# NAIVEddd/MafrixRaytracing

Hardware: AMD Instinct MI355X
Metric: Mrays/s (primary+secondary) at 1080p/64spp; 1/2/4/8-GPU scaling (higher is better)
Workload: dtype f64; 1 GPU; C2 spot (5856 tris) + floor/light stage, 1920x1080, 64 spp per step over 1 GPU(s); scene=scenes/spot.xml, width=1920, height=1080, max_depth=3, frames_in_flight=1, pipeline=wavefront, api=mfx_trace_accumulate of the step's spp (inputs resident in HBM), parallelism=one GPU

## Files before the change

mafrixraytracing_amd/csrc/cut_check.cpp:

```cpp
#include <algorithm>
#include <cfloat>
#include <cinttypes>
#include <cmath>
#include <cstdio>
#include <cstdlib>
#include <cstring>
#include <string>
#include <vector>

#include "mfx_build.h"
#include "mfx_camera_cuts.h"
#include "mfx_scene.h"

hipError_t mfx_gpu_build_images(const float*, const float*, const int32_t*, int, int, float, const MfxGpuLayoutIn&,
                                MfxGpuImages&) {
    return hipErrorNotSupported;
}

namespace {

struct Rng {
    uint64_t x;
    uint64_t next() {
        uint64_t z = (x += 0x9e3779b97f4a7c15ULL);
        z = (z ^ (z >> 30)) * 0xbf58476d1ce4e5b9ULL;
        z = (z ^ (z >> 27)) * 0x94d049bb133111ebULL;
        return z ^ (z >> 31);
    }
    double unit() { return (double)(next() >> 11) * 0x1p-53; }
    double in(double lo, double hi) { return lo + (hi - lo) * unit(); }
};

const double ALBEDO[9] = {0.75, 0.25, 0.25, 0.25, 0.75, 0.25, 0.5, 0.5, 0.5};

mfx_pinhole pinhole(double px, double py, double pz, double dx, double dy, double dz, double fov) {
    mfx_pinhole c;
    std::memset(&c, 0, sizeof(c));
    c.position[0] = px; c.position[1] = py; c.position[2] = pz;
    c.direction[0] = dx; c.direction[1] = dy; c.direction[2] = dz;
    c.fov = fov;
    c.aspect = 16.0 / 9.0;
    return c;
}

mfx_scene_desc desc_of(const std::vector<mfx_prim>& prims, const mfx_pinhole& cam) {
    mfx_scene_desc d;
    std::memset(&d, 0, sizeof(d));
    d.prims = prims.data();
    d.nprims = (int64_t)prims.size();
    d.albedo = ALBEDO;
    d.nmat = 3;
    d.width = 40;
    d.height = 24;
    d.max_depth = 3;
    const double q[4][3] = {{-0.5, 2.5, -0.5}, {0.5, 2.5, -0.5}, {0.5, 2.5, 0.5}, {-0.5, 2.5, 0.5}};
    std::memcpy(d.light.p, q, sizeof(q));
    d.light.normal[1] = -1.0;
    d.light.intensity[0] = d.light.intensity[1] = d.light.intensity[2] = 3.0;
    d.camera = cam;
    return d;
}

std::vector<mfx_prim> soup(int n, uint64_t seed) {
    Rng r{seed};
    std::vector<mfx_prim> v(n);
    for (int i = 0; i < n; ++i) {
        mfx_prim& p = v[i];
        std::memset(&p, 0, sizeof(p));
        p.material = i % 3;
        const double x = r.in(-1.0, 1.0), y = r.in(-1.0, 1.0), z = r.in(-1.0, 1.0);
        if (i % 3 == 0) {
            p.kind = MFX_PRIM_TRIANGLE;
            const double c[3] = {x, y, z};
            for (int k = 0; k < 3; ++k)
                for (int a = 0; a < 3; ++a) p.p[k][a] = c[a] + (k ? r.in(-0.05, 0.05) : 0.0);
        } else if (i % 3 == 1) {
            p.kind = MFX_PRIM_RECT;
            const double u = r.in(0.02, 0.1), w = r.in(0.02, 0.1), t = r.in(-0.03, 0.03);
            const double q[4][3] = {{x, y, z}, {x + u, y, z + t}, {x + u, y + w, z + t}, {x, y + w, z}};
            std::memcpy(p.p, q, sizeof(q));
        } else {
            p.kind = MFX_PRIM_SPHERE;
            p.p[0][0] = x; p.p[0][1] = y; p.p[0][2] = z;
            p.p[1][0] = r.in(0.01, 0.08);
        }
    }
    return v;
}

bool load_prims(const char* path, std::vector<mfx_prim>& v) {
    FILE* f = std::fopen(path, "rb");
    if (!f) return false;
    std::fseek(f, 0, SEEK_END);
    const long bytes = std::ftell(f);
    std::fseek(f, 0, SEEK_SET);
    if (bytes <= 0 || bytes % (long)sizeof(mfx_prim) != 0) {
        std::fclose(f);
        return false;
    }
    v.resize((size_t)bytes / sizeof(mfx_prim));
    const size_t got = std::fread(v.data(), sizeof(mfx_prim), v.size(), f);
    std::fclose(f);
    return got == v.size();
}

struct RayF {
    float ix, iy, iz, oix, oiy, oiz;
};
RayF make_rayf(const double* o, const double* d) {
    float dx = (float)d[0], dy = (float)d[1], dz = (float)d[2];
    const float tiny = 1e-20f;
    if (std::fabs(dx) < tiny) dx = std::copysign(tiny, dx);
    if (std::fabs(dy) < tiny) dy = std::copysign(tiny, dy);
    if (std::fabs(dz) < tiny) dz = std::copysign(tiny, dz);
    RayF r;
    r.ix = 1.0f / dx; r.iy = 1.0f / dy; r.iz = 1.0f / dz;
    r.oix = (float)o[0] * r.ix; r.oiy = (float)o[1] * r.iy; r.oiz = (float)o[2] * r.iz;
    return r;
}
bool slab(const MfxNode& nd, int k, const RayF& r, float& n) {
    const float a0 = std::fmaf(nd.lox[k], r.ix, -r.oix), a1 = std::fmaf(nd.hix[k], r.ix, -r.oix);
    const float b0 = std::fmaf(nd.loy[k], r.iy, -r.oiy), b1 = std::fmaf(nd.hiy[k], r.iy, -r.oiy);
    const float c0 = std::fmaf(nd.loz[k], r.iz, -r.oiz), c1 = std::fmaf(nd.hiz[k], r.iz, -r.oiz);
    n = std::fmax(std::fmax(std::fmin(a0, a1), std::fmin(b0, b1)), std::fmax(std::fmin(c0, c1), 0.0f));
    const float f = std::fmin(std::fmin(std::fmax(a0, a1), std::fmax(b0, b1)), std::fmin(std::fmax(c0, c1), FLT_MAX));
    return n <= f;
}

struct Totals {
    long long rays = 0, leaves = 0, uncovered = 0, lb_above = 0, tiles = 0, root = 0, empty = 0, multi = 0;
};

int find_entry(const MfxCutEntry* row, int cap, int code) {
    for (int i = 0; i < cap && row[i].code != MFX_CUT_END; ++i)
        if (row[i].code == code) return i;
    return -1;
}

void check_ray(const std::vector<MfxNode>& nodes, const RayF& r, const MfxCutEntry* row, int cap, Totals& t) {
    struct Item {
        int node, cov;
    };
    std::vector<Item> stack{{0, find_entry(row, cap, 0)}};
    while (!stack.empty()) {
        const Item it = stack.back();
        stack.pop_back();
        const MfxNode& nd = nodes[it.node];
        for (int k = 0; k < 4; ++k) {
            if (nd.child[k] == MFX_CHILD_EMPTY) continue;
            float n = 0.f;
            if (!slab(nd, k, r, n)) continue;
            int cov = it.cov;
            if (cov < 0) {
                cov = find_entry(row, cap, nd.child[k]);
                if (cov >= 0 && !(row[cov].lb <= n)) ++t.lb_above;
            }
            if (nd.child[k] >= 0) {
                stack.push_back({nd.child[k], cov});
            } else {
                ++t.leaves;
                if (cov < 0) ++t.uncovered;
            }
        }
    }
}

void check_case(const char* scene, const char* camname, const MfxHostScene& s, const MfxCamera& cam, int W, int H, int cap,
                Totals& all, double* root_share = nullptr) {
    const int tiles_x = (W + 7) / 8, tiles_y = (H + 7) / 8;
    std::vector<MfxCutEntry> table((size_t)tiles_x * tiles_y * cap);
    MfxCutStats st;
    mfx_cut::table_host(s.nodes.data(), cam, W, H, cap, table.data(), st);
    Totals t;
    t.tiles = (long long)tiles_x * tiles_y;
    t.root = (long long)st.root_tiles;
    t.empty = (long long)st.empty_tiles;
    for (int n = 2; n <= MFX_CUT_CAP_MAX; ++n) t.multi += (long long)st.hist[n];
    Rng jr{(uint64_t)(W * 131 + H * 7 + cap)};
    const double one = 1.0 - 0x1p-53;
    for (int y = 0; y < H; ++y)
        for (int x = 0; x < W; ++x) {
            const MfxCutEntry* row = table.data() + (size_t)((y / 8) * tiles_x + x / 8) * cap;
            for (int j = 0; j < 16; ++j) {
                const double ju = j < 4 ? ((j & 1) ? one : 0.0) : jr.unit(), jv = j < 4 ? ((j & 2) ? one : 0.0) : jr.unit();
                const double u = ((double)x + ju) / (double)W, v = ((double)y + jv) / (double)H;
                double o[3], d[3];
                for (int a = 0; a < 3; ++a) {
                    o[a] = cam.position[a];
                    d[a] = ((cam.topleft[a] + cam.right[a] * u) + cam.down[a] * v) - o[a];
                }
                const double l = std::sqrt(d[0] * d[0] + d[1] * d[1] + d[2] * d[2]);
                if (l != 0.0)
                    for (int a = 0; a < 3; ++a) d[a] = d[a] / l;
                ++t.rays;
                check_ray(s.nodes, make_rayf(o, d), row, cap, t);
            }
        }
    std::printf("%s %s %dx%d cap=%d: tiles=%lld root=%lld empty=%lld multi=%lld mean_len=%.3f max_len=%llu rays=%lld leaves=%lld"
                " uncovered=%lld lb_above=%lld\n",
                scene, camname, W, H, cap, t.tiles, t.root, t.empty, t.multi, (double)st.len_sum / (double)t.tiles, st.len_max,
                t.rays, t.leaves, t.uncovered, t.lb_above);
    if (root_share) *root_share = (double)t.root / (double)t.tiles;
    all.rays += t.rays; all.leaves += t.leaves; all.uncovered += t.uncovered; all.lb_above += t.lb_above;
    all.tiles += t.tiles; all.root += t.root; all.empty += t.empty; all.multi += t.multi;
}

bool build(const std::vector<mfx_prim>& prims, const mfx_pinhole& cam, MfxHostScene& s) {
    const mfx_scene_desc d = desc_of(prims, cam);
    std::string err;
    if (!mfx_build_scene(&d, s, err)) {
        std::printf("build FAILED: %s\n", err.c_str());
        return false;
    }
    return true;
}

struct NamedCam {
    const char* name;
    mfx_pinhole cam;
};

std::vector<NamedCam> cameras(const mfx_pinhole& def, const MfxHostScene& s) {
    double c[3], R = 0.0;
    for (int a = 0; a < 3; ++a) {
        c[a] = 0.5 * (s.box_lo[a] + s.box_hi[a]);
        R = std::max(R, 0.5 * (s.box_hi[a] - s.box_lo[a]));
    }
    const double* p = def.position;
    const double* d = def.direction;
    const double dl = std::sqrt(d[0] * d[0] + d[1] * d[1] + d[2] * d[2]);
    return {{"default", def},
            {"inside", pinhole(c[0], c[1], c[2], d[0], d[1], d[2], 90.0)},
            {"away", pinhole(p[0], p[1], p[2], -d[0], -d[1], -d[2], 90.0)},
            {"axis", pinhole(c[0], c[1], c[2] + 3.0 * R, 0.0, 0.0, -1.0, 90.0)},
            {"far_0.6deg", pinhole(c[0] - 200.0 * R * d[0] / dl, c[1] - 200.0 * R * d[1] / dl, c[2] - 200.0 * R * d[2] / dl, d[0],
                                   d[1], d[2], 0.6)},
            {"fov120", pinhole(p[0], p[1], p[2], d[0], d[1], d[2], 120.0)}};
}

int check_scene(const char* name, const std::vector<mfx_prim>& prims, const mfx_pinhole& def, bool cap_root_share, Totals& all) {
    MfxHostScene s;
    if (!build(prims, def, s)) return 1;
    int bad = 0;
    for (const NamedCam& nc : cameras(def, s)) {
        MfxCamera cam;
        mfx_derive_camera(nc.cam, cam);
        const int films[2][2] = {{40, 24}, {17, 9}};
        for (const auto& f : films)
            for (const int cap : {MFX_CUT_CAP_DEFAULT, 1, 2, MFX_CUT_CAP_MAX}) {
                double share = 0.0;
                check_case(name, nc.name, s, cam, f[0], f[1], cap, all, &share);
                if (cap_root_share && cap == MFX_CUT_CAP_DEFAULT && std::strcmp(nc.name, "default") == 0) {
                    std::printf("%s default %dx%d: {root} share %.4f (cap 0.05)\n", name, f[0], f[1], share);
                    if (share > 0.05) {
                        std::printf("FAIL: {root} share above 5 %%\n");
                        ++bad;
                    }
                }
            }
    }
    return bad;
}

int distribution(const std::vector<mfx_prim>& prims, const mfx_pinhole& def, int W, int H) {
    MfxHostScene s;
    if (!build(prims, def, s)) return 1;
    MfxCamera cam;
    mfx_derive_camera(def, cam);
    const int tiles = ((W + 7) / 8) * ((H + 7) / 8);
    for (const int cap : {MFX_CUT_CAP_MAX, MFX_CUT_CAP_DEFAULT}) {
        std::vector<MfxCutEntry> table((size_t)tiles * cap);
        MfxCutStats st;
        mfx_cut::table_host(s.nodes.data(), cam, W, H, cap, table.data(), st);
        long long internal = 0, entries = 0;
        for (const MfxCutEntry& e : table)
            if (e.code != MFX_CUT_END) {
                ++entries;
                internal += e.code >= 0;
            }
        std::printf("%dx%d cap=%d nodes=%zu tiles=%d mean=%.3f max=%llu root=%llu empty=%llu internal_entries=%.4f hist:", W, H, cap,
                    s.nodes.size(), tiles, (double)st.len_sum / tiles, st.len_max, st.root_tiles, st.empty_tiles,
                    entries ? (double)internal / (double)entries : 0.0);
        for (int n = 0; n <= cap; ++n) std::printf(" %d:%llu", n, st.hist[n]);
        std::printf("\n");
    }
    return 0;
}

}

int main(int argc, char** argv) {
    const mfx_pinhole spot_cam = pinhole(2.4, 1.3, -3.4, -2.4, -1.2, 3.4, 90.0);
    const mfx_pinhole soup_cam = pinhole(0.0, 0.0, 4.5, 0.0, 0.0, -1.0, 90.0);
    std::vector<mfx_prim> mesh;
    if (argc > 1 && !load_prims(argv[1], mesh)) {
        std::printf("cannot read %s\n", argv[1]);
        return 2;
    }
    if (argc == 4) return distribution(mesh, spot_cam, std::atoi(argv[2]), std::atoi(argv[3]));
    if (argc == 11) {
        double v[7];
        for (int i = 0; i < 7; ++i) v[i] = std::atof(argv[4 + i]);
        return distribution(mesh, pinhole(v[0], v[1], v[2], v[3], v[4], v[5], v[6]), std::atoi(argv[2]), std::atoi(argv[3]));
    }
    Totals all;
    int bad = check_scene("soup_600", soup(600, 600), soup_cam, false, all);
    if (!mesh.empty()) bad += check_scene("mesh", mesh, spot_cam, true, all);
    std::printf("total: rays=%lld leaves=%lld uncovered=%lld lb_above=%lld tiles=%lld root=%lld empty=%lld multi=%lld\n", all.rays,
                all.leaves, all.uncovered, all.lb_above, all.tiles, all.root, all.empty, all.multi);
    if (all.uncovered || all.lb_above) {
        std::printf("FAIL: a reached leaf is not covered, or an entry's lb is above a ray's entry distance\n");
        ++bad;
    }
    if (all.empty == 0 || all.multi == 0 || all.leaves == 0) {
        std::printf("FAIL: vacuous (no empty cut, no cut of more than one entry, or no leaf reached)\n");
        ++bad;
    }
    return bad ? 1 : 0;
}
```

mafrixraytracing_amd/csrc/mfx_api.cpp:

```cpp
#include <dlfcn.h>

#include <set>
#include <thread>

#include "mfx_ctx.h"
#include "mfx_half.h"

using namespace mfxh;

namespace {
thread_local std::string g_err;

using mfx_half::node_to_half;

template <typename T>
hipError_t upload(DevBuf<T>& d, const std::vector<T>& v) {
    const hipError_t e = d.alloc(std::max<size_t>(1, v.size()));
    if (e != hipSuccess || v.empty()) return e;
    return hipMemcpy(d, v.data(), v.size() * sizeof(T), hipMemcpyHostToDevice);
}
}

int mfxh::fail(int code, const std::string& msg) {
    g_err = msg;
    return code;
}

const Rccl* mfxh::rccl() {
    static Rccl r;
    static bool tried = false, ok = false;
    if (tried) return ok ? &r : nullptr;
    tried = true;
    void* h = dlopen("librccl.so.1", RTLD_NOW | RTLD_GLOBAL);
    if (!h) h = dlopen("/opt/rocm/lib/librccl.so.1", RTLD_NOW | RTLD_GLOBAL);
    if (!h) return nullptr;
    r.commInitAll = (decltype(r.commInitAll))dlsym(h, "ncclCommInitAll");
    r.commDestroy = (decltype(r.commDestroy))dlsym(h, "ncclCommDestroy");
    r.reduce = (decltype(r.reduce))dlsym(h, "ncclReduce");
    r.groupStart = (decltype(r.groupStart))dlsym(h, "ncclGroupStart");
    r.groupEnd = (decltype(r.groupEnd))dlsym(h, "ncclGroupEnd");
    r.errorString = (decltype(r.errorString))dlsym(h, "ncclGetErrorString");
    ok = r.commInitAll && r.commDestroy && r.reduce && r.groupStart && r.groupEnd && r.errorString;
    return ok ? &r : nullptr;
}

int mfxh::whole_film_single_device(const mfx_ctx* c, const char* who) {
    if (c->api_part_count != 1 || (c->flags & MFX_F_ROW_PARTITION) || c->multi.device_list || !c->multi.peers.empty())
        return fail(MFX_E_STATE, std::string(who) + " needs one device and the whole film and sample set "
                                                    "(no device list, part_count == 1, no MFX_F_ROW_PARTITION)");
    return MFX_OK;
}

mfx_ctx::~mfx_ctx() {
    for (ncclComm_t cm : multi.comms)
        if (cm) (void)rccl()->commDestroy(cm);
    multi.comms.clear();
    multi.peers.clear();
    (void)hipSetDevice(device);
}

static CreateEnv read_create_env() {
    const auto set = [](const char* name) { return getenv(name) != nullptr; };
    const auto num = [](const char* name) { return getenv(name) ? CreateEnv::Int(atoi(getenv(name))) : std::nullopt; };
    CreateEnv v;
    v.node_f32 = set("MFX_NODE_F32");
    v.diag_iter = set("MFX_DIAG_ITER");
    v.no_gray_light = set("MFX_NO_GRAY_LIGHT");
    v.no_lit_in_hit = set("MFX_NO_LIT_IN_HIT");
    v.mega_waves = num("MFX_MEGA_WAVES");
    v.shadow_target_blocks = num("MFX_SHADOW_TARGET_BLOCKS");
    v.stack_lds = num("MFX_STACK_LDS");
    v.ntop = num("MFX_NTOP");
    v.slot_lds = num("MFX_SLOT_LDS");
    v.shadow_waves = num("MFX_SHADOW_WAVES");
    v.blocks_per_cu = num("MFX_BLOCKS_PER_CU");
    v.camera_packets = num("MFX_CAMERA_PACKETS");
    v.cam_blocks = num("MFX_CAM_BLOCKS");
    v.camera_cuts = num("MFX_CAMERA_CUTS");
    v.camera_cut_cap = num("MFX_CAMERA_CUT_CAP");
    v.camera_cut_min_samples = num("MFX_CAMERA_CUT_MIN_SAMPLES");
    v.pool_fail_once = num("MFX_POOL_FAIL_ONCE");
    v.adaptive_check = num("MFX_ADAPTIVE_CHECK");
    v.iter_events = num("MFX_ITER_EVENTS");
    v.queue_from = num("MFX_QUEUE_FROM");
    v.qchunk = num("MFX_QCHUNK");
    v.ray_queue = num("MFX_RAY_QUEUE");
    v.mega_chunk = num("MFX_MEGA_CHUNK");
    v.shd_half = num("MFX_SHD_HALF");
    v.chunk = num("MFX_CHUNK");
    if (const char* e = getenv("MFX_POOL")) v.pool = atoll(e);
    return v;
}

template <typename F>
static int largest_keeping(int lo, int hi, F keeps) {
    while (lo < hi) {
        const int mid = (lo + hi + 1) / 2;
        if (keeps(mid)) lo = mid;
        else hi = mid - 1;
    }
    return lo;
}

#define CK(expr) HIP_TRY(expr, _e == hipErrorOutOfMemory ? MFX_E_NOMEM : MFX_E_DEVICE, #expr ": ")

static int scene_upload(mfx_ctx* c) {
    c->image_gen += 1;
    c->stack_size = std::max(1, c->host.stack_entries);
    if (c->stack_size > 96) return fail(MFX_E_INVALID, "mfx_create: BVH too deep for the LDS traversal stack");
    CK(upload(c->d_nodes, c->host.nodes));
    CK(upload(c->d_slots, c->host.slots));
    if (MFX_NODE_F16 && !c->env.node_f32) {
        std::vector<MfxNodeH> nh(c->host.nodes.size());
        for (size_t i = 0; i < nh.size(); ++i) nh[i] = node_to_half(c->host.nodes[i]);
        CK(upload(c->d_nodes_h, nh));
    }
    CK(upload(c->d_slot_ref, c->host.slot_ref));
    CK(upload(c->d_ref_blob, c->host.ref_blob));
    CK(upload(c->d_shade, c->host.shade));
    CK(upload(c->d_albedo, c->host.albedo));
    CK(upload(c->d_light, std::vector<MfxLight>{c->host.light}));
    if (wf_multi_light(c)) CK(upload(c->d_lights, c->host.lights));
    else c->d_lights.reset();
    CK(upload(c->d_cam, std::vector<MfxCamera>{c->host.camera}));
    CK(upload(c->d_refs, std::vector<const void*>{c->d_slot_ref.get(), c->d_ref_blob.get()}));
    if (!c->host.inst.empty()) CK(upload(c->d_inst, c->host.inst));
    else c->d_inst.reset();
    return MFX_OK;
}

static int scene_shapes(mfx_ctx* c) {
    const CreateEnv& env = c->env;
    const bool inst = !c->host.inst.empty();
    hipDeviceProp_t prop;
    CK(hipGetDeviceProperties(&prop, c->device));
    int bpc = 0;
    c->mega_waves = c->stack_size <= 36 ? 4 : 1;
    if (env.mega_waves) c->mega_waves = *env.mega_waves == 4 ? 4 : 1;
    CK(mfx_trace_occupancy(c->stack_size, &bpc, inst, c->mega_waves));
    bpc = std::max(1, std::min(bpc, 8));
    c->grid = prop.multiProcessorCount * bpc;
    WfParams& A = c->pool.params;
    hipError_t qerr = hipSuccess;
    auto blocks = [&](bool shd, int nlds, int ntop = 0, int nslot = 0) {
        const WfLdsShape s{shd, nlds < c->stack_size, c->d_nodes_h != nullptr, nlds, ntop, (int)c->host.inst.size(), nslot,
                           shd && wf_multi_light(c)};
        int b = 0;
        const hipError_t e = mfx_wf_kernel_occupancy(s, &b);
        if (e != hipSuccess && qerr == hipSuccess) qerr = e;
        return e == hipSuccess ? b : 0;
    };
    int ebpc = 0, sbpc = 0;
    for (const bool shd : {false, true}) {
        const int full = blocks(shd, c->stack_size);
        int nlds = c->stack_size;
        if (c->stack_size > WF_STACK_LDS) {
            const int b16 = blocks(shd, WF_STACK_LDS);
            const int target = shd ? std::max(full, std::min(env.shadow_target_blocks.value_or(8), b16)) : b16;
            if (full < target) nlds = largest_keeping(WF_STACK_LDS, c->stack_size - 1, [&](int n) { return blocks(shd, n) >= target; });
            if (c->diag_iter)
                fprintf(stderr, "wavefront: %s blocks/CU: full %d-entry stacks %d, %d in LDS %d; chosen %d in LDS, %d\n",
                        shd ? "k_shadow" : "k_extend", c->stack_size, full, WF_STACK_LDS, b16, nlds, blocks(shd, nlds));
        }
        if (env.stack_lds) nlds = std::max(1, std::min(c->stack_size, *env.stack_lds));
        (shd ? A.stack_lds_shd : A.stack_lds_ext) = nlds;
        (shd ? sbpc : ebpc) = blocks(shd, nlds);
    }
    {
        int cap = std::min((int)c->host.nodes.size(), WF_NTOP_MAX);
        if (env.ntop) cap = std::max(0, std::min(cap, *env.ntop));
        for (const bool shd : {false, true}) {
            const int nlds = shd ? A.stack_lds_shd : A.stack_lds_ext, want = shd ? sbpc : ebpc;
            const int ntop = largest_keeping(0, cap, [&](int n) { return blocks(shd, nlds, n) >= want; });
            (shd ? A.ntop_shd : A.ntop_ext) = ntop;
            int ns = inst ? 0 : (int)c->host.slots.size();
            if (ns > WF_SLOT_LDS_MAX || (env.slot_lds && *env.slot_lds == 0)) ns = 0;
            if (ns > 0 && blocks(shd, nlds, ntop, ns) < want) ns = 0;
            (shd ? A.nslot_shd : A.nslot_ext) = ns;
        }
        HIP_TRY(qerr, MFX_E_DEVICE, "mfx_wf_kernel_occupancy: ");
        A.shadow_waves = sbpc <= 3 ? 3 : 4;
        if (env.shadow_waves) A.shadow_waves = *env.shadow_waves == 3 ? 3 : 4;
        if (wf_multi_light(c)) A.shadow_waves = 4;
        if (A.shadow_waves == 3) sbpc = std::min(sbpc, 3);
        if (c->diag_iter)
            fprintf(stderr,
                    "wavefront: stack %d/%d (extend) %d/%d (shadow) in LDS, blocks/CU extend %d shadow %d (%d-wave "
                    "build), top nodes in LDS %d / %d, slots in LDS %d / %d\n",
                    A.stack_lds_ext, c->stack_size, A.stack_lds_shd, c->stack_size, ebpc, sbpc,
                    A.shadow_waves, A.ntop_ext, A.ntop_shd, A.nslot_ext, A.nslot_shd);
    }
    if (env.blocks_per_cu) {
        ebpc = std::min(ebpc, std::max(1, *env.blocks_per_cu));
        sbpc = std::min(sbpc, std::max(1, *env.blocks_per_cu));
    }
    c->wf_ext_grid = prop.multiProcessorCount * std::max(1, std::min(ebpc, 8));
    {
        if (env.camera_packets.value_or(1) && !inst) {
            int cb = 0;
            c->cuts.on = env.camera_cuts.value_or(1) != 0;
            c->cuts.cap = std::max(1, std::min(env.camera_cut_cap.value_or(MFX_CUT_CAP_DEFAULT), MFX_CUT_CAP_MAX));
            c->cuts.min_samples = std::max(1, env.camera_cut_min_samples.value_or(MFX_CUT_MIN_SAMPLES));
            CK(mfx_cam_occupancy(c->stack_size, &cb, c->cuts.on));
            if (env.cam_blocks) cb = std::min(cb, std::max(1, *env.cam_blocks));
            c->wf_cam_grid = prop.multiProcessorCount * std::max(1, std::min(cb, 8));
        }
    }
    c->wf_shd_grid = prop.multiProcessorCount * std::max(1, std::min(sbpc, 8));
    {
        const size_t lanes = (size_t)std::max(c->wf_ext_grid, c->wf_shd_grid) * 256;
        const int deep = c->stack_size - std::min(A.stack_lds_ext, A.stack_lds_shd);
        CK(c->d_spill.alloc(lanes * std::max(1, deep)));
        c->spill_deep = std::max(1, deep);
        c->spill_lanes = (int)lanes;
    }
    CK(c->d_vscratch.alloc(6 * (size_t)(c->host.max_depth + 1) * c->grid * 256));
    return MFX_OK;
}

static int ctx_setup(mfx_ctx* c) {
    c->npix = (int64_t)c->host.width * c->host.height;
    const CreateEnv& env = c->env = read_create_env();
    CK(hipSetDevice(c->device));
    CK(c->stream.create());
    CK(c->h_counters.alloc(WF_NCTR * WF_SHARDS));
    CK(c->ev0.create());
    CK(c->ev1.create());
    MFX_TRY(scene_upload(c));
    const size_t npix = (size_t)c->npix, plane = sizeof(double) * npix;
    CK(c->d_accum_own.alloc(3 * npix));
    c->d_accum = c->d_accum_own;
    CK(c->d_film.alloc(3 * npix));
    CK(c->d_frame.alloc(4 * npix));
    CK(c->d_rgba.alloc(4 * npix));
    CK(c->d_work.alloc(8));
    CK(c->d_counters.alloc(WF_NCTR * WF_SHARDS));
    CK(c->d_counters_total.alloc(WF_NCTR * WF_SHARDS));
    CK(hipMemset(c->d_counters_total, 0, kCounterBytes));
    CK(c->pool.ctl.alloc(WF_CTL_ALLOC));
    size_t mfree = 0, mtotal = 0;
    if (hipMemGetInfo(&mfree, &mtotal) == hipSuccess && mfree > 0)
        c->pool.max = std::max<int64_t>(1 << 20, std::min<int64_t>(c->pool.max, (int64_t)(mfree / 4 / pool_slot_bytes(c))));
    c->pool.fail_once = env.pool_fail_once.value_or(0) != 0;
    if (env.pool) c->pool.max = std::max<int64_t>(2048, std::min<int64_t>(1 << 28, *env.pool));
    c->diag_iter = env.diag_iter;
    c->adp.check = env.adaptive_check.value_or(0) != 0;
    if (env.iter_events) c->iter_events = *env.iter_events != 0 || c->diag_iter;
    if (env.queue_from) c->pool.queue_from = MFX_RAY_QUEUE ? std::max(-2, *env.queue_from) : -1;
    if (env.qchunk) c->pool.qchunk = std::max(64, std::min(WF_CHUNK_MAX, *env.qchunk / 64 * 64));
    if (env.ray_queue && *env.ray_queue == 0) c->pool.queue_from = -1;
    if (env.mega_chunk) c->mega_chunk = std::max(1, *env.mega_chunk);
    if (c->flags & MFX_F_IN_FLIGHT) {
        c->wf_chunk = 512;
        c->wf_shd_half = false;
    }
    if (env.shd_half) c->wf_shd_half = *env.shd_half != 0;
    if (env.chunk) c->wf_chunk = std::max(64, std::min(WF_CHUNK_MAX, *env.chunk / 64 * 64));
    CK(hipMemset(c->d_accum, 0, 3 * plane));
    CK(hipMemset(c->d_film, 0, 3 * plane));
    CK(hipMemset(c->d_counters, 0, kCounterBytes));
    return scene_shapes(c);
}
#undef CK

static bool flatten_instances(const mfx_scene_desc* scene, const mfx_instance* instances, int32_t ninstances,
                              int32_t flags, size_t device_free = 0) {
    if (flags & MFX_F_FLATTEN) return true;
    if (!instances || (flags & MFX_F_TWO_LEVEL)) return false;
    double budget = 2.0 * 1024 * 1024 * 1024;
    if (const char* e = getenv("MFX_FLATTEN_MAX_BYTES")) budget = atof(e);
    if (device_free > 0) budget = std::min(budget, (double)device_free / 16.0);
    double slots = 0.0;
    for (int32_t i = 0; i < ninstances; ++i) {
        const int64_t f = instances[i].first, n = instances[i].count;
        if (f < 0 || n < 0 || f + n > scene->nprims) return false;
        for (int64_t k = f; k < f + n; ++k) slots += scene->prims[k].kind == MFX_PRIM_RECT ? 2.0 : 1.0;
    }
    return slots * 512.0 <= budget;
}

static hipError_t repeated_device_setup(mfx_ctx* c) {
    hipError_t e = hipSetDevice(c->device);
    if (e == hipSuccess) e = c->multi.reduce_stage.alloc(3 * (size_t)c->npix);
    if (e == hipSuccess) e = c->multi.reduce_done.create(hipEventDisableTiming);
    if (e != hipSuccess) return e;
    for (const auto& p : c->multi.peers) {
        Event ev;
        if ((e = hipSetDevice(p->device)) != hipSuccess) return e;
        if ((e = ev.create(hipEventDisableTiming)) != hipSuccess) return e;
        c->multi.peer_done.push_back(std::move(ev));
    }
    return hipSetDevice(c->device);
}

static_assert(WF_MAX_LIGHTS == MFX_MAX_LIGHTS, "the kernels' light index width is the ABI's bound");

static int create_impl(const mfx_scene_desc* scene, const mfx_instance* instances, int32_t ninstances,
                       const mfx_options* opt, mfx_ctx** out, const mfx_quad_light* lights = nullptr, int32_t nlights = 0) {
    if (!scene || !opt || !out) return fail(MFX_E_INVALID, "mfx_create: null argument");
    *out = nullptr;
    std::vector<MfxLight> prepared;
    if (lights) {
        std::string lerr;
        if (!mfx_prepare_lights(lights, nlights, prepared, lerr)) return fail(MFX_E_INVALID, "mfx_create_lights: " + lerr);
        if (nlights >= 2 && (opt->flags & (MFX_F_MEGAKERNEL | MFX_F_COUNT_STATS)))
            return fail(MFX_E_INVALID, "mfx_create_lights: MFX_F_MEGAKERNEL and MFX_F_COUNT_STATS need a single light");
    }
    if (opt->part_count < 1 || opt->part_index < 0 || opt->part_index >= opt->part_count)
        return fail(MFX_E_INVALID, "mfx_create: bad sample partition");
    if (opt->ndevices < 0 || opt->ndevices > MFX_MAX_DEVICES || (opt->ndevices > 0 && !opt->devices))
        return fail(MFX_E_INVALID, "mfx_create: bad device list");
    if (opt->render_ahead < 0 || opt->render_ahead > MFX_MAX_RENDER_AHEAD)
        return fail(MFX_E_INVALID, "mfx_create: render_ahead out of range");
    if (scene->nmat > WF_MAT_MAX) return fail(MFX_E_INVALID, "mfx_create: more than 65,536 materials");
    if ((opt->flags & MFX_F_FLATTEN) && (opt->flags & MFX_F_TWO_LEVEL))
        return fail(MFX_E_INVALID, "mfx_create: MFX_F_FLATTEN and MFX_F_TWO_LEVEL exclude each other");
    int ndev = 0;
    HIPCHECK(hipGetDeviceCount(&ndev));
    std::vector<int> devlist;
    if (opt->ndevices == 0) devlist.push_back(opt->device);
    else devlist.assign(opt->devices, opt->devices + opt->ndevices);
    for (int d : devlist)
        if (d < 0 || d >= ndev) return fail(MFX_E_DEVICE, "mfx_create: no such HIP device");
    const int G = (int)devlist.size();
    HIPCHECK(hipSetDevice(devlist[0]));
    size_t dev_free = 0, dev_total = 0;
    if (hipMemGetInfo(&dev_free, &dev_total) != hipSuccess) dev_free = 0;
    std::unique_ptr<mfx_ctx> c(new mfx_ctx());
    c->device = devlist[0];
    std::string err;
    const bool flatten = flatten_instances(scene, instances, ninstances, opt->flags, dev_free);
    if (!mfx_build_scene(scene, c->host, err, (opt->flags & MFX_F_HOST_BVH) == 0, instances, ninstances, flatten, lights,
                         lights ? &prepared : nullptr)) {
        const bool dev = err.rfind("GPU BVH build", 0) == 0;
        return fail(dev ? MFX_E_DEVICE : MFX_E_INVALID, "mfx_create: " + err);
    }
    {
        KeptScene& k = c->kept;
        k.prims.assign(scene->prims, scene->prims + scene->nprims);
        k.albedo.assign(scene->albedo, scene->albedo + 3 * (size_t)scene->nmat);
        if (instances) k.instances.assign(instances, instances + ninstances);
        if (lights) k.lights.assign(lights, lights + nlights);
        k.desc = *scene;
        k.desc.prims = nullptr;
        k.desc.albedo = nullptr;
        k.instanced = instances != nullptr;
        k.flatten = flatten;
        k.gpu_bvh = (opt->flags & MFX_F_HOST_BVH) == 0;
    }
    const bool rows = (opt->flags & MFX_F_ROW_PARTITION) != 0;
    auto init = [&](mfx_ctx* d, int g) {
        d->device = devlist[g];
        d->seed = opt->seed;
        d->flags = opt->flags;
        d->part_index = rows ? 0 : opt->part_index;
// ... 215 lines not shown
    return n;
}

int mfx_create(const mfx_scene_desc* scene, const mfx_options* opt, mfx_ctx** out) {
    return create_impl(scene, nullptr, 0, opt, out);
}

int mfx_create_instanced(const mfx_scene_desc* scene, const mfx_instance* instances, int32_t ninstances,
                         const mfx_options* opt, mfx_ctx** out) {
    if (!instances || ninstances < 1) return fail(MFX_E_INVALID, "mfx_create_instanced: no instances");
    return create_impl(scene, instances, ninstances, opt, out);
}

int mfx_create_lights(const mfx_scene_desc* scene, const mfx_quad_light* lights, int32_t nlights,
                      const mfx_instance* instances, int32_t ninstances, const mfx_options* opt, mfx_ctx** out) {
    if (!lights || nlights < 1 || nlights > MFX_MAX_LIGHTS)
        return fail(MFX_E_INVALID, "mfx_create_lights: nlights must be 1 .. MFX_MAX_LIGHTS with a light array");
    const bool flat = !instances && ninstances == 0;
    if (!flat && (!instances || ninstances < 1)) return fail(MFX_E_INVALID, "mfx_create_lights: no instances");
    return create_impl(scene, instances, flat ? 0 : ninstances, opt, out, lights, nlights);
}

int mfx_light_table(const mfx_quad_light* lights, int32_t nlights, double* out) {
    if (!out) return fail(MFX_E_INVALID, "mfx_light_table: null argument");
    std::vector<MfxLight> t;
    std::string err;
    if (!mfx_prepare_lights(lights, nlights, t, err)) return fail(MFX_E_INVALID, "mfx_light_table: " + err);
    for (int32_t n = 0; n < nlights; ++n) {
        out[4 * n + 0] = t[n].area;
        out[4 * n + 1] = 1. / t[n].area;
        out[4 * n + 2] = t[n].pdf;
        out[4 * n + 3] = 0.0;
    }
    return MFX_OK;
}

int mfx_light_info(mfx_ctx* c, double out[8]) {
    if (!c || !out) return fail(MFX_E_INVALID, "mfx_light_info: null argument");
    const bool ml = wf_multi_light(c);
    const WfParams& A = c->pool.params;
    HIPCHECK(hipSetDevice(c->device));
    const WfLdsShape s{true, A.stack_lds_shd < c->stack_size, c->d_nodes_h != nullptr, A.stack_lds_shd, A.ntop_shd,
                       (int)c->host.inst.size(), A.nslot_shd, ml};
    int sb = 0, rb = 0;
    HIPCHECK(mfx_wf_kernel_occupancy(s, &sb));
    if (A.shadow_waves == 3) sb = std::min(sb, 3);
    HIPCHECK(mfx_wf_resolve_occupancy(ml, &rb));
    const double v[8] = {(double)c->host.lights.size(), ml ? 1.0 : 0.0, ml ? (double)(c->host.lights.size() * sizeof(MfxLight)) : 0.0,
                         ml ? (double)WF_LIGHT_BYTES_PER_SLOT(c->host.max_depth + 1) : 0.0, (double)sb, (double)rb, 0.0, 0.0};
    std::copy(v, v + 8, out);
    return MFX_OK;
}

void mfx_destroy(mfx_ctx* ctx) { delete ctx; }

int mfx_expand_instances(const mfx_prim* prims, int64_t nprims, const mfx_instance* instances, int32_t ninstances,
                         mfx_prim* out, int64_t cap, int64_t* nout) {
    if (!nout) return fail(MFX_E_INVALID, "mfx_expand_instances: null count");
    std::vector<mfx_prim> w;
    std::string err;
    if (!mfx_expand(prims, nprims, instances, ninstances, w, err)) return fail(MFX_E_INVALID, "mfx_expand_instances: " + err);
    *nout = (int64_t)w.size();
    if (out) {
        if (cap < (int64_t)w.size()) return fail(MFX_E_INVALID, "mfx_expand_instances: output too small");
        std::copy(w.begin(), w.end(), out);
    }
    return MFX_OK;
}

int mfx_instancing_info(mfx_ctx* c, double out[8]) {
    if (!c || !out) return fail(MFX_E_INVALID, "null argument");
    instancing_info(c->host, out);
    return MFX_OK;
}

int mfx_build_instanced_info(const mfx_scene_desc* scene, const mfx_instance* instances, int32_t ninstances,
                             int32_t flags, double out[8], int32_t* stack_entries) {
    if (!out) return fail(MFX_E_INVALID, "null argument");
    MfxHostScene h;
    std::string err;
    if (!scene) return fail(MFX_E_INVALID, "null argument");
    if ((flags & MFX_F_FLATTEN) && (flags & MFX_F_TWO_LEVEL))
        return fail(MFX_E_INVALID, "mfx_build_instanced_info: MFX_F_FLATTEN and MFX_F_TWO_LEVEL exclude each other");
    if (!mfx_build_scene(scene, h, err, false, instances, ninstances, flatten_instances(scene, instances, ninstances, flags)))
        return fail(MFX_E_INVALID, "mfx_build_instanced_info: " + err);
    instancing_info(h, out);
    if (stack_entries) *stack_entries = h.stack_entries;
    return MFX_OK;
}

int mfx_build_info(mfx_ctx* c, double out[8], uint64_t* digest) {
    if (!c) return fail(MFX_E_STATE, "null context");
    const MfxHostScene& h = c->host;
    if (out) {
        out[0] = h.ms_ref_bvh;
        out[1] = h.ms_bvh;
        out[2] = h.ms_total;
        out[3] = h.images_gpu ? 2.0 : (h.bvh_gpu ? 1.0 : 0.0);
        out[4] = (double)h.nodes.size();
        out[5] = (double)h.slots.size();
        out[6] = h.nodes2;
        out[7] = h.bvh_levels;
    }
    if (digest) *digest = mfx_scene_digest(h);
    return MFX_OK;
}

int mfx_device_info(mfx_ctx* c, int32_t* out, int32_t cap) {
    if (!c || !out) return fail(MFX_E_INVALID, "null argument");
    const std::vector<mfx_ctx*> ds = devs_of(c);
    if (cap < 5 + (int32_t)ds.size()) return fail(MFX_E_INVALID, "mfx_device_info: cap < 5 + devices");
    out[0] = (int32_t)ds.size();
    out[1] = (int32_t)c->multi.comms.size();
    out[2] = !c->multi.comms.empty() ? 1 : (c->multi.peers.empty() ? 0 : 2);
    out[3] = c->band_index;
    out[4] = c->band_count;
    for (size_t g = 0; g < ds.size(); ++g) out[5 + g] = ds[g]->device;
    return MFX_OK;
}

int mfx_launch_info(mfx_ctx* c, int32_t* out, int32_t cap) {
    if (!c || !out) return fail(MFX_E_INVALID, "null argument");
    if (cap < MFX_LAUNCH_INFO_N) return fail(MFX_E_INVALID, "mfx_launch_info: cap < MFX_LAUNCH_INFO_N");
    const WfParams& A = c->pool.params;
    const bool inst = !c->host.inst.empty();
    const bool cuts = cuts_apply(c);
    if (cuts) MFX_TRY(cuts_read_stats(c));
    const CamCuts& K = c->cuts;
    const int64_t tiles = (int64_t)((c->host.width + 7) / 8) * ((c->host.height + 7) / 8);
    const int32_t v[MFX_LAUNCH_INFO_N] = {
        c->stack_size, A.stack_lds_ext, A.stack_lds_shd, A.stack_lds_ext < c->stack_size, A.stack_lds_shd < c->stack_size,
        A.ntop_ext, A.ntop_shd, A.nslot_ext, A.nslot_shd, inst ? std::min<int>((int)c->host.inst.size(), WF_INST_LDS) : 0,
        A.shadow_waves, c->mega_waves, wf_lit_in_hit(c), wf_gray_light(c), !inst && c->wf_cam_grid > 0,
        c->wf_ext_grid, c->wf_shd_grid, inst ? 0 : c->wf_cam_grid, c->spill_deep, c->spill_lanes,
        c->wf_chunk, c->wf_shd_half, c->pool.queue_from, (int32_t)std::min<int64_t>(c->pool.max, INT32_MAX),
        cuts, cuts ? K.cap : 0, cuts ? (int32_t)std::min<int64_t>(tiles * K.cap * (int64_t)sizeof(MfxCutEntry), INT32_MAX) : 0,
        (int32_t)(K.last.len_sum * 1000 / (unsigned long long)std::max<int64_t>(1, tiles)), (int32_t)K.last.len_max,
        (int32_t)K.last.root_tiles, (int32_t)std::min<int64_t>(K.builds, INT32_MAX), cuts ? K.min_samples : 0};
    std::copy(v, v + MFX_LAUNCH_INFO_N, out);
    return MFX_OK;
}

int mfx_camera_cut_table(mfx_ctx* c, void* out, int64_t cap_bytes, int64_t* nbytes, int32_t host) {
    if (!c || !nbytes) return fail(MFX_E_INVALID, "mfx_camera_cut_table: null argument");
    if (!cuts_apply(c)) return fail(MFX_E_STATE, "mfx_camera_cut_table: the context does not use camera cuts");
    const size_t tiles = (size_t)((c->host.width + 7) / 8) * (size_t)((c->host.height + 7) / 8);
    const size_t bytes = tiles * c->cuts.cap * sizeof(MfxCutEntry);
    *nbytes = (int64_t)bytes;
    if (!out) return MFX_OK;
    if (cap_bytes < (int64_t)bytes) return fail(MFX_E_INVALID, "mfx_camera_cut_table: output too small");
    if (host) {
        std::vector<MfxCutEntry> t(tiles * c->cuts.cap);
        MfxCutStats st;
        mfx_cut::table_host(c->host.nodes.data(), c->host.camera, c->host.width, c->host.height, c->cuts.cap, t.data(), st);
        std::memcpy(out, t.data(), bytes);
        return MFX_OK;
    }
    HIPCHECK(hipSetDevice(c->device));
    MFX_TRY(cuts_ensure(c));
    HIPCHECK(hipMemcpyAsync(out, c->cuts.table, bytes, hipMemcpyDeviceToHost, c->stream));
    HIPCHECK(hipStreamSynchronize(c->stream));
    return MFX_OK;
}

int mfx_camera_cut_info(mfx_ctx* c, double out[32]) {
    if (!c || !out) return fail(MFX_E_INVALID, "mfx_camera_cut_info: null argument");
    for (int k = 0; k < 32; ++k) out[k] = 0.0;
    if (!cuts_apply(c)) return MFX_OK;
    MFX_TRY(cuts_read_stats(c));
    const CamCuts& K = c->cuts;
    out[0] = (double)K.builds;
    out[1] = (double)K.last_ms;
    out[2] = (double)K.last.len_sum;
    out[3] = (double)K.last.len_max;
    out[4] = (double)K.last.root_tiles;
    out[5] = (double)K.last.empty_tiles;
    out[6] = (double)((int64_t)((c->host.width + 7) / 8) * ((c->host.height + 7) / 8));
    out[7] = (double)K.cap;
    for (int n = 0; n <= MFX_CUT_CAP_MAX; ++n) out[8 + n] = (double)K.last.hist[n];
    return MFX_OK;
}

int mfx_stats(mfx_ctx* c, double* rays, double* seconds) {
    if (!c) return fail(MFX_E_INVALID, "null context");
    if (seconds) {
        double ms = 0;
        MFX_TRY(mfx_last_trace_ms(c, &ms));
        *seconds = ms * 1e-3;
    }
    if (rays) {
        double n[16];
        MFX_TRY(mfx_ray_counts(c, n));
        *rays = n[0] + n[1] + n[2];
    }
    return MFX_OK;
}

int mfx_reset(mfx_ctx* c) {
    if (!c) return fail(MFX_E_STATE, "null context");
    for (mfx_ctx* d : devs_of(c)) {
        HIPCHECK(hipSetDevice(d->device));
        HIPCHECK(hipMemsetAsync(d->d_film, 0, 3 * sizeof(double) * (size_t)d->npix, d->stream));
    }
    HIPCHECK(hipSetDevice(c->device));
    c->frame_count = 0.0;
    c->ahead.film_in_dfilm = true;
    c->ahead.dfilm_buf = -1;
    if (c->ahead.ready()) {
        c->ahead.film_epoch += 1;
        c->ahead.cur = -1;
        return MFX_OK;
    }
    return mfx_sync(c);
}

int mfx_sync(mfx_ctx* c) {
    if (!c) return fail(MFX_E_STATE, "null context");
    for (mfx_ctx* d : devs_of(c)) {
        HIPCHECK(hipSetDevice(d->device));
        HIPCHECK(hipStreamSynchronize(d->stream));
    }
    return MFX_OK;
}

int mfx_stream(mfx_ctx* c, void** stream) {
    if (!c || !stream) return fail(MFX_E_INVALID, "null argument");
    *stream = (void*)c->stream.get();
    return MFX_OK;
}
}
```

mafrixraytracing_amd/csrc/mfx_build.h:

```cpp
#ifndef MFX_BUILD_H
#define MFX_BUILD_H

#include <hip/hip_runtime.h>
#include <stdint.h>

#include <vector>

#include "mfx_camera_cuts.h"
#include "mfx_layout.h"

struct MfxGpuLayoutIn {
    const MfxSlot* pslots;
    const MfxShade* pshade;
    const int32_t* slot_of;
    const int32_t* ref16_of;
    int32_t nslots;
    int32_t top_nodes;
};
struct MfxGpuImages {
    std::vector<MfxNode> nodes;
    std::vector<MfxSlot> slots;
    std::vector<int32_t> slot_ref;
    std::vector<MfxShade> shade;
    std::vector<int32_t> shade_of;
    int32_t max_depth = 0, max_stack = 0, nodes2 = 0, nleaves = 0, levels = 0;
};
hipError_t mfx_gpu_build_images(const float* prim_box, const float* cent, const int32_t* weight, int n, int max_leaf,
                                float c_isect, const MfxGpuLayoutIn& in, MfxGpuImages& out);

hipError_t mfx_build_cut_table(const MfxNode* nodes, const MfxCamera* cam_dev, int W, int H, int cap, MfxCutEntry* table,
                               MfxCutStats* stats_dev, hipStream_t st);

#endif
```

mafrixraytracing_amd/csrc/mfx_build.hip:

```cpp
#include <float.h>
#include <hip/hip_runtime.h>
#include <stdint.h>

#include <algorithm>
#include <numeric>

#include "mfx_build.h"
#include "mfx_camera_cuts.h"

namespace {

constexpr int NB = 32;

struct BTask {
    int b, e, parent, side;
};

struct BArgs {
    const float* __restrict__ box;
    const float* __restrict__ cent;
    const int* __restrict__ weight;
    int* ids;
    int* tmp;
    float* node_box;
// ... 479 lines not shown
    ok(dalloc(&D.d_weight, (size_t)n));
    ok(dalloc(&A.ids, (size_t)n));
    ok(dalloc(&A.tmp, (size_t)n));
    ok(dalloc(&A.node_box, 12 * (size_t)n));
    ok(dalloc(&A.node_child, 2 * (size_t)n));
    ok(dalloc(&A.leaves, (size_t)n));
    ok(dalloc(&A.counters, 4));
    ok(dalloc(&A.root_box, 6));
    ok(dalloc(&A.root_ref, 1));
    ok(dalloc(&D.t0, (size_t)n));
    ok(dalloc(&D.t1, (size_t)n));
    if (e == hipSuccess) {
        ok(hipMemcpy(D.d_box, prim_box, sizeof(float) * 6 * (size_t)n, hipMemcpyHostToDevice));
        ok(hipMemcpy(D.d_cent, cent, sizeof(float) * 3 * (size_t)n, hipMemcpyHostToDevice));
        ok(hipMemcpy(D.d_weight, weight, sizeof(int) * (size_t)n, hipMemcpyHostToDevice));
        ok(hipMemcpy(A.ids, iota.data(), sizeof(int) * (size_t)n, hipMemcpyHostToDevice));
        ok(hipMemset(A.counters, 0, 4 * sizeof(int)));
        const BTask root{0, n, -1, 0};
        ok(hipMemcpy(D.t0, &root, sizeof(BTask), hipMemcpyHostToDevice));
    }
    A.box = D.d_box;
    A.cent = D.d_cent;
    A.weight = D.d_weight;
    A.max_leaf = max_leaf;
    A.c_isect = c_isect;
    int ntasks = 1;
    while (e == hipSuccess && ntasks > 0) {
        ok(hipMemset(A.counters + 2, 0, sizeof(int)));
        hipLaunchKernelGGL(k_sah_level, dim3((ntasks + 3) / 4), dim3(256), 0, 0, A, D.t0, ntasks, D.t1);
        ok(hipGetLastError());
        ok(hipMemcpy(&ntasks, A.counters + 2, sizeof(int), hipMemcpyDeviceToHost));
        std::swap(D.t0, D.t1);
        ++D.levels;
        if (D.levels > 4 * 64 + n) ok(hipErrorUnknown);
    }
    int cnt[2] = {0, 0};
    ok(hipMemcpy(cnt, A.counters, 2 * sizeof(int), hipMemcpyDeviceToHost));
    ok(hipMemcpy(&D.root, A.root_ref, sizeof(int), hipMemcpyDeviceToHost));
    D.nodes = cnt[0];
    D.nleaves = cnt[1];
    return e;
}

hipError_t mfx_gpu_build_images(const float* prim_box, const float* cent, const int32_t* weight, int n, int max_leaf,
                                float c_isect, const MfxGpuLayoutIn& in, MfxGpuImages& out) {
    DevBvh2 D;
    hipError_t e = bvh2_build(prim_box, cent, weight, n, max_leaf, c_isect, D);
    auto ok = [&](hipError_t r) {
        if (e == hipSuccess) e = r;
        return e == hipSuccess;
    };
    const int n4max = D.nodes + 1;
    W4* W = nullptr;
    int *F = nullptr, *cnt = nullptr, *total = nullptr, *slot_of = nullptr, *ref16 = nullptr, *shade_of = nullptr;
    int *size = nullptr, *nsl = nullptr, *pre = nullptr, *sstart = nullptr, *pushed = nullptr, *lstart = nullptr,
        *idx = nullptr, *mstack = nullptr;
    MfxSlot *pslots = nullptr, *slots = nullptr;
    MfxShade *pshade = nullptr, *shade = nullptr;
    MfxNode* nodes = nullptr;
    int32_t* slot_ref = nullptr;
    const size_t ns = (size_t)in.nslots;
    ok(dalloc(&W, n4max));
    ok(dalloc(&F, n4max));
    ok(dalloc(&cnt, n4max));
    ok(dalloc(&total, 1));
    ok(dalloc(&size, n4max));
    ok(dalloc(&nsl, n4max));
    ok(dalloc(&pre, n4max));
    ok(dalloc(&sstart, n4max));
    ok(dalloc(&pushed, n4max));
    ok(dalloc(&idx, n4max));
    ok(dalloc(&mstack, 1));
    ok(dalloc(&lstart, (size_t)std::max(1, D.nleaves)));
    ok(dalloc(&slot_of, (size_t)n + 1));
    ok(dalloc(&ref16, (size_t)n));
    ok(dalloc(&shade_of, (size_t)n));
    ok(dalloc(&pslots, ns));
    ok(dalloc(&pshade, ns));
    ok(dalloc(&slots, ns + MFX_LEAF_SLOTS_MAX));
    ok(dalloc(&slot_ref, ns));
    ok(dalloc(&shade, ns));
    ok(dalloc(&nodes, n4max));
    if (e == hipSuccess) {
        ok(hipMemcpy(slot_of, in.slot_of, sizeof(int) * ((size_t)n + 1), hipMemcpyHostToDevice));
        ok(hipMemcpy(ref16, in.ref16_of, sizeof(int) * (size_t)n, hipMemcpyHostToDevice));
        ok(hipMemcpy(pslots, in.pslots, sizeof(MfxSlot) * ns, hipMemcpyHostToDevice));
        ok(hipMemcpy(pshade, in.pshade, sizeof(MfxShade) * ns, hipMemcpyHostToDevice));
        ok(hipMemset(slots + ns, 0, sizeof(MfxSlot) * MFX_LEAF_SLOTS_MAX));
        ok(hipMemcpy(F, &D.root, sizeof(int), hipMemcpyHostToDevice));
        ok(hipMemset(pre, 0, sizeof(int)));
        ok(hipMemset(sstart, 0, sizeof(int)));
        ok(hipMemset(pushed, 0, sizeof(int)));
        ok(hipMemset(mstack, 0, sizeof(int)));
    }
    std::vector<int> lo;
    int base = 0, nF = 1;
    while (e == hipSuccess && nF > 0) {
        if (base + nF > n4max) {
            ok(hipErrorUnknown);
            break;
        }
        lo.push_back(base);
        const dim3 g((nF + 255) / 256);
        hipLaunchKernelGGL(k_collapse, g, dim3(256), 0, 0, F + base, nF, D.A.node_box, D.A.node_child, D.A.root_box,
                           W + base, cnt + base);
        hipLaunchKernelGGL(k_scan, dim3(1), dim3(1024), 0, 0, cnt + base, nF, total);
        hipLaunchKernelGGL(k_frontier, g, dim3(256), 0, 0, W + base, nF, cnt + base, base + nF, F + base + nF);
        ok(hipGetLastError());
        int t = 0;
        ok(hipMemcpy(&t, total, sizeof(int), hipMemcpyDeviceToHost));
        base += nF;
        nF = t;
    }
    const int n4 = base;
    lo.push_back(n4);
    const int nlev = (int)lo.size() - 1;
    LArgs A{W, D.A.leaves, D.A.ids, slot_of, size, nsl, pre, sstart, pushed, lstart, idx, mstack};
    for (int L = nlev - 1; L >= 0 && e == hipSuccess; --L)
        hipLaunchKernelGGL(k_sizes, dim3((lo[L + 1] - lo[L] + 255) / 256), dim3(256), 0, 0, A, lo[L], lo[L + 1]);
    for (int L = 0; L < nlev && e == hipSuccess; ++L)
        hipLaunchKernelGGL(k_preorder, dim3((lo[L + 1] - lo[L] + 255) / 256), dim3(256), 0, 0, A, lo[L], lo[L + 1]);
    if (e == hipSuccess && n4 > 0) {
        hipLaunchKernelGGL(k_index, dim3((n4 + 255) / 256), dim3(256), 0, 0, A, n4, in.top_nodes);
        hipLaunchKernelGGL(k_nodes, dim3((n4 + 255) / 256), dim3(256), 0, 0, A, n4, nodes);
        hipLaunchKernelGGL(k_slots, dim3((D.nleaves + 255) / 256), dim3(256), 0, 0, A, D.nleaves, pslots, pshade, ref16,
                           slots, slot_ref, shade, shade_of);
        ok(hipGetLastError());
    }
    if (e == hipSuccess) {
        out.nodes.resize(n4);
        out.slots.resize(ns + MFX_LEAF_SLOTS_MAX);
        out.slot_ref.resize(ns);
        out.shade.resize(ns);
        out.shade_of.resize(n);
        ok(hipMemcpy(out.nodes.data(), nodes, sizeof(MfxNode) * n4, hipMemcpyDeviceToHost));
        ok(hipMemcpy(out.slots.data(), slots, sizeof(MfxSlot) * out.slots.size(), hipMemcpyDeviceToHost));
        ok(hipMemcpy(out.slot_ref.data(), slot_ref, sizeof(int32_t) * ns, hipMemcpyDeviceToHost));
        ok(hipMemcpy(out.shade.data(), shade, sizeof(MfxShade) * ns, hipMemcpyDeviceToHost));
        ok(hipMemcpy(out.shade_of.data(), shade_of, sizeof(int32_t) * (size_t)n, hipMemcpyDeviceToHost));
        ok(hipMemcpy(&out.max_stack, mstack, sizeof(int), hipMemcpyDeviceToHost));
        out.max_depth = nlev - 1;
        out.nodes2 = D.nodes;
        out.nleaves = D.nleaves;
        out.levels = D.levels;
    }
    void* bufs[] = {W, F, cnt, total, size, nsl, pre, sstart, pushed, idx, mstack, lstart, slot_of, ref16, shade_of,
                    pslots, pshade, slots, slot_ref, shade, nodes};
    for (void* p : bufs)
        if (p) (void)hipFree(p);
    bvh2_free(D);
    return e;
}

__global__ void __launch_bounds__(64) k_cut_table(const MfxNode* __restrict__ nodes, const MfxCamera* __restrict__ cam, int W, int H,
                                                  int tiles_x, int ntiles, int cap, MfxCutEntry* __restrict__ table,
                                                  MfxCutStats* __restrict__ stats) {
    __shared__ MfxCutEntry lists[MFX_CUT_CAP_MAX * 64];
    const int t = blockIdx.x * blockDim.x + threadIdx.x;
    const bool valid = t < ntiles;
    int n = -1;
    bool root = false;
    if (valid) {
        MfxCutEntry* row = table + (size_t)t * cap;
        n = mfx_cut::tile_cut(nodes, *cam, W, H, t % tiles_x, t / tiles_x, cap, row, lists + threadIdx.x, 64);
        root = n == 1 && row[0].code == 0;
    }
    int sum = valid ? n : 0, mx = sum;
    for (int off = 32; off > 0; off >>= 1) {
        sum += __shfl_xor(sum, off);
        mx = max(mx, __shfl_xor(mx, off));
    }
    const unsigned long long roots = __popcll(__ballot(root));
    for (int v = 0; v <= cap; ++v) {
        const unsigned long long cnt = __popcll(__ballot(n == v));
        if (threadIdx.x == 0 && cnt) {
            atomicAdd(&stats->hist[v], cnt);
            if (v == 0) atomicAdd(&stats->empty_tiles, cnt);
        }
    }
    if (threadIdx.x == 0) {
        atomicAdd(&stats->len_sum, (unsigned long long)sum);
        atomicMax(&stats->len_max, (unsigned long long)mx);
        if (roots) atomicAdd(&stats->root_tiles, roots);
    }
}

hipError_t mfx_build_cut_table(const MfxNode* nodes, const MfxCamera* cam_dev, int W, int H, int cap, MfxCutEntry* table,
                               MfxCutStats* stats_dev, hipStream_t st) {
    const int tiles_x = (W + 7) / 8, ntiles = tiles_x * ((H + 7) / 8);
    if (cap < 1 || cap > MFX_CUT_CAP_MAX || ntiles < 1) return hipErrorInvalidValue;
    const hipError_t e = hipMemsetAsync(stats_dev, 0, sizeof(MfxCutStats), st);
    if (e != hipSuccess) return e;
    hipLaunchKernelGGL(k_cut_table, dim3((ntiles + 63) / 64), dim3(64), 0, st, nodes, cam_dev, W, H, tiles_x, ntiles, cap, table,
                       stats_dev);
    return hipGetLastError();
}
```

mafrixraytracing_amd/csrc/mfx_camera_cuts.h:

```cpp
#ifndef MFX_CAMERA_CUTS_H
#define MFX_CAMERA_CUTS_H

#include <math.h>
#include <stdint.h>

#include "mfx_layout.h"

#if defined(__HIPCC__)
#define MFX_CUT_HD __host__ __device__ inline
#else
#define MFX_CUT_HD inline
#endif

#define MFX_CUT_CAP_MAX 16
#define MFX_CUT_CAP_DEFAULT 8
#define MFX_CUT_END (-0x7fffffff - 1)
#define MFX_CUT_MIN_GAP 0x1p-16
#define MFX_CUT_MARGIN 0x1p-17
#define MFX_CUT_MIN_SAMPLES 32

struct alignas(32) MfxCutEntry {
    int32_t code;
    float lb;
    float lo[3], hi[3];
};

struct MfxCutStats {
    unsigned long long len_sum, len_max, root_tiles, empty_tiles, hist[MFX_CUT_CAP_MAX + 1];
};

namespace mfx_cut {

struct V3 {
    double x, y, z;
};
MFX_CUT_HD V3 v3(const double* p) { return {p[0], p[1], p[2]}; }
MFX_CUT_HD V3 add(V3 a, V3 b) { return {a.x + b.x, a.y + b.y, a.z + b.z}; }
MFX_CUT_HD V3 sub(V3 a, V3 b) { return {a.x - b.x, a.y - b.y, a.z - b.z}; }
MFX_CUT_HD V3 mul(V3 a, double s) { return {a.x * s, a.y * s, a.z * s}; }
MFX_CUT_HD double dot(V3 a, V3 b) { return a.x * b.x + a.y * b.y + a.z * b.z; }
MFX_CUT_HD V3 cross(V3 a, V3 b) { return {a.y * b.z - a.z * b.y, a.z * b.x - a.x * b.z, a.x * b.y - a.y * b.x}; }
MFX_CUT_HD double max2(double a, double b) { return a > b ? a : b; }
MFX_CUT_HD double abs1(double a) { return a < 0.0 ? -a : a; }
MFX_CUT_HD bool finite1(double a) { return a - a == 0.0; }

MFX_CUT_HD V3 film_dir(const MfxCamera& cam, double px, double py, int W, int H) {
    const double u = px / (double)W, v = py / (double)H;
    const V3 target = add(add(v3(cam.topleft), mul(v3(cam.right), u)), mul(v3(cam.down), v));
    return sub(target, v3(cam.position));
}

struct Pyramid {
    V3 n[4];
    V3 pos;
    double mpos;
    bool ok;
};

MFX_CUT_HD Pyramid pyramid_of(const MfxCamera& cam, int W, int H, int tx, int ty) {
    Pyramid P;
    P.pos = v3(cam.position);
    P.mpos = max2(abs1(P.pos.x), max2(abs1(P.pos.y), abs1(P.pos.z)));
    P.ok = true;
    const int x0 = tx * 8, y0 = ty * 8;
    const int x1 = x0 + 8 < W ? x0 + 8 : W, y1 = y0 + 8 < H ? y0 + 8 : H;
    const V3 c00 = film_dir(cam, x0 - 1, y0 - 1, W, H), c01 = film_dir(cam, x1 + 1, y0 - 1, W, H);
    const V3 c10 = film_dir(cam, x0 - 1, y1 + 1, W, H), c11 = film_dir(cam, x1 + 1, y1 + 1, W, H);
    const V3 mid = add(add(c00, c01), add(c10, c11));
    const V3 raw[4] = {cross(c00, c10), cross(c01, c11), cross(c00, c01), cross(c10, c11)};
    for (int k = 0; k < 4; ++k) {
        V3 n = raw[k];
        const double l2 = dot(n, n);
        if (!(l2 > 0.0) || !finite1(l2)) {
            P.ok = false;
            n = V3{0.0, 0.0, 0.0};
        } else {
            const double l = sqrt(l2);
            n = mul(n, (dot(n, mid) < 0.0 ? -1.0 : 1.0) / l);
        }
        P.n[k] = n;
    }
    const V3 in[4] = {film_dir(cam, x0, y0, W, H), film_dir(cam, x1, y0, W, H), film_dir(cam, x0, y1, W, H),
                      film_dir(cam, x1, y1, W, H)};
    for (int i = 0; i < 4; ++i) {
        const double l2 = dot(in[i], in[i]);
        if (!(l2 > 0.0) || !finite1(l2)) {
            P.ok = false;
            continue;
        }
        const double l = sqrt(l2);
        for (int k = 0; k < 4; ++k)
            if (!(dot(P.n[k], in[i]) / l >= MFX_CUT_MIN_GAP)) P.ok = false;
    }
    return P;
}

MFX_CUT_HD double box_mag(const float* lo, const float* hi) {
    double m = 0.0;
    for (int a = 0; a < 3; ++a) m = max2(m, max2(abs1((double)lo[a]), abs1((double)hi[a])));
    return m;
}

MFX_CUT_HD bool outside(const Pyramid& P, const float* lo, const float* hi) {
    const double m = MFX_CUT_MARGIN * (box_mag(lo, hi) + P.mpos);
    if (!finite1(m)) return false;
    const double p[3] = {P.pos.x, P.pos.y, P.pos.z};
    for (int k = 0; k < 4; ++k) {
        const double n[3] = {P.n[k].x, P.n[k].y, P.n[k].z};
        double s = 0.0;
        for (int a = 0; a < 3; ++a) s += max2(n[a] * ((double)lo[a] - p[a]), n[a] * ((double)hi[a] - p[a]));
        if (s < -m) return true;
    }
    return false;
}

MFX_CUT_HD float lower_bound(const Pyramid& P, const float* lo, const float* hi) {
    const double p[3] = {P.pos.x, P.pos.y, P.pos.z};
    double d2 = 0.0;
    for (int a = 0; a < 3; ++a) {
        const double d = max2(max2((double)lo[a] - p[a], p[a] - (double)hi[a]), 0.0);
        d2 += d * d;
    }
    if (!(d2 > 0.0)) return 0.0f;
    const double dist = sqrt(d2);
    const double lb = dist - (dist * 0x1p-20 + MFX_CUT_MARGIN * (box_mag(lo, hi) + P.mpos));
    if (!(lb > 0.0) || !finite1(lb)) return 0.0f;
    float f = (float)lb;
    if ((double)f > lb) f = nextafterf(f, 0.0f);
    return f;
}

MFX_CUT_HD MfxCutEntry root_entry() {
    return MfxCutEntry{0, 0.0f, {-3.402823466e38f, -3.402823466e38f, -3.402823466e38f},
                       {3.402823466e38f, 3.402823466e38f, 3.402823466e38f}};
}

MFX_CUT_HD int tile_cut(const MfxNode* nodes, const MfxCamera& cam, int W, int H, int tx, int ty, int cap, MfxCutEntry* row,
                        MfxCutEntry* list, int stride) {
    cap = cap < 1 ? 1 : (cap > MFX_CUT_CAP_MAX ? MFX_CUT_CAP_MAX : cap);
    int n = 1;
    list[0] = root_entry();
    const Pyramid P = pyramid_of(cam, W, H, tx, ty);
    uint64_t need = 0;
    bool changed = P.ok;
    while (changed) {
        changed = false;
        for (int i = 0; i < n;) {
            const int code = list[i * stride].code;
            const int known = (int)((need >> (4 * i)) & 15);
            if (code < 0 || (known && n - 1 + known > cap)) {
                ++i;
                continue;
            }
            const MfxNode& nd = nodes[code];
            int k = 0;
            unsigned keep = 0;
            for (int c = 0; c < 4; ++c) {
                if (nd.child[c] == MFX_CHILD_EMPTY) continue;
                const float lo[3] = {nd.lox[c], nd.loy[c], nd.loz[c]}, hi[3] = {nd.hix[c], nd.hiy[c], nd.hiz[c]};
                if (outside(P, lo, hi)) continue;
                keep |= 1u << c;
                ++k;
            }
            if (n - 1 + k > cap) {
                need = (need & ~((uint64_t)15 << (4 * i))) | ((uint64_t)k << (4 * i));
                ++i;
                continue;
            }
            --n;
            list[i * stride] = list[n * stride];
            need = (need & ~((uint64_t)15 << (4 * i))) | (((need >> (4 * n)) & 15) << (4 * i));
            for (int c = 0; c < 4; ++c) {
                if (!((keep >> c) & 1)) continue;
                MfxCutEntry e;
                e.code = nd.child[c];
                e.lo[0] = nd.lox[c]; e.lo[1] = nd.loy[c]; e.lo[2] = nd.loz[c];
                e.hi[0] = nd.hix[c]; e.hi[1] = nd.hiy[c]; e.hi[2] = nd.hiz[c];
                e.lb = lower_bound(P, e.lo, e.hi);
                need &= ~((uint64_t)15 << (4 * n));
                list[n * stride] = e;
                ++n;
            }
            changed = true;
        }
    }
    for (int i = 1; i < n; ++i) {
        const MfxCutEntry e = list[i * stride];
        int j = i;
        while (j > 0 && (list[(j - 1) * stride].lb > e.lb || (list[(j - 1) * stride].lb == e.lb && list[(j - 1) * stride].code > e.code))) {
            list[j * stride] = list[(j - 1) * stride];
            --j;
        }
        list[j * stride] = e;
    }
    for (int i = 0; i < cap; ++i) row[i] = i < n ? list[i * stride] : MfxCutEntry{MFX_CUT_END, 0.0f, {0.0f, 0.0f, 0.0f}, {0.0f, 0.0f, 0.0f}};
    return n;
}
inline int tile_cut(const MfxNode* nodes, const MfxCamera& cam, int W, int H, int tx, int ty, int cap, MfxCutEntry* row) {
    MfxCutEntry list[MFX_CUT_CAP_MAX];
    return tile_cut(nodes, cam, W, H, tx, ty, cap, row, list, 1);
}

MFX_CUT_HD void count_tile(MfxCutStats& s, int n, const MfxCutEntry* row) {
    s.len_sum += (unsigned long long)n;
    if ((unsigned long long)n > s.len_max) s.len_max = (unsigned long long)n;
    if (n == 1 && row[0].code == 0) s.root_tiles += 1;
    if (n == 0) s.empty_tiles += 1;
    s.hist[n] += 1;
}

inline void table_host(const MfxNode* nodes, const MfxCamera& cam, int W, int H, int cap, MfxCutEntry* table, MfxCutStats& stats) {
    const int tiles_x = (W + 7) / 8, tiles_y = (H + 7) / 8;
    stats = MfxCutStats{};
    for (int ty = 0; ty < tiles_y; ++ty)
        for (int tx = 0; tx < tiles_x; ++tx) {
            MfxCutEntry* row = table + (size_t)(ty * tiles_x + tx) * cap;
            count_tile(stats, tile_cut(nodes, cam, W, H, tx, ty, cap, row), row);
        }
}

}

#endif
```

mafrixraytracing_amd/csrc/mfx_ctx.h:

```cpp
#pragma once
#include <hip/hip_runtime.h>
#include <rccl/rccl.h>

#include <algorithm>
#include <cmath>
#include <cstdio>
#include <cstdlib>
#include <cstring>
#include <functional>
#include <memory>
#include <optional>
#include <string>
#include <utility>
#include <variant>
#include <vector>

#include "../../include/mafrix_rt.h"
#include "mfx_device.h"
#include "mfx_denoise.h"
#include "mfx_scene.h"
#include "mfx_wavefront.h"

namespace mfxh __attribute__((visibility("hidden"))) {

// ... 65 lines not shown

constexpr size_t kCounterBytes = WF_NCTR * WF_SHARDS * sizeof(unsigned long long);

struct AheadBuf {
    DevBuf<uint8_t> frames;
    DevBuf<double> film_in;
    DevBuf<double> film_out;
    DevBuf<unsigned long long> counters;
    Event t0, t1;
    Event ready;
    int64_t base = 0, n = 0;
    int64_t expect = 0;
    uint64_t epoch = 0;
    double count0 = 0.0;
    bool reported = false;
};

struct FrameMode {
    double* film;
    uint8_t* frames;
    double count0;
    unsigned long long* counters;
    hipEvent_t e0, e1;
};

struct ResolveSplit {
    int nbands = 0;
    std::function<int(int, int, int)> after;
    bool used = false;
};

struct TileList {
    const int32_t* tiles;
    int32_t ntiles;
    double* mom;
    int64_t gen_paths;
    const int32_t* tile_n = nullptr;
    int32_t list_max = 0;
};

using TraceMode = std::variant<std::monostate, FrameMode, ResolveSplit*, TileList>;

constexpr int kStageChunks = 8;

struct Rccl {
    decltype(&ncclCommInitAll) commInitAll = nullptr;
    decltype(&ncclCommDestroy) commDestroy = nullptr;
    decltype(&ncclReduce) reduce = nullptr;
    decltype(&ncclGroupStart) groupStart = nullptr;
    decltype(&ncclGroupEnd) groupEnd = nullptr;
    decltype(&ncclGetErrorString) errorString = nullptr;
};
const Rccl* rccl();

struct WfPool {
    WfParams params{};
    DevBuf<char> mem;
    int32_t slots = 0;
    size_t bytes = 0;
    bool queues = false;
    WfQueue wq[2]{};
    int queue_from = MFX_RAY_QUEUE ? -2 : -1;
    int queue_auto = 1;
    bool auto_read = false;
    bool auto_pending = false;
    int32_t qchunk = 128;
    int64_t max = 1 << 28;
    int64_t cap = 0;
    bool fail_once = false;
    DevBuf<unsigned long long> ctl;
    int queue_start() const { return queue_from == -2 ? queue_auto : queue_from; }
};

struct Ahead {
    int k = 0;
    AheadBuf ab[2];
    int nbuf = 0;
    int cap = 0;
    int cur = -1;
    int64_t last_k = -1;
    uint64_t film_epoch = 1;
    bool film_in_dfilm = true;
    int dfilm_buf = -1;
    int64_t dfilm_n = 0;
    DevBuf<unsigned long long> counters_aux;
    Event aux_ev0, aux_ev1;
    bool ready() const { return nbuf != 0; }
    void release() {
        for (AheadBuf& B : ab) B = AheadBuf{};
        counters_aux.reset(), aux_ev0.reset(), aux_ev1.reset();
        nbuf = cap = 0;
        cur = -1;
    }
};

struct Adaptive {
    DevBuf<double> mom;
    DevBuf<int32_t> tiles[2];
    DevBuf<int32_t> tile_flags;
    DevBuf<int32_t> tile_spp;
    DevBuf<int32_t> tile_count;
    Event ev0, ev1;
    bool check = false;
    bool accum_valid = false;
    int64_t B = 0;
    int32_t R = 0;
    int64_t gen_paths = 0;
    bool ready() const { return ev1 != nullptr; }
};

struct Denoise {
    DevBuf<double> feat;
    DevBuf<double> feat_out;
    DevBuf<double> buf[2];
    DevBuf<double> var[2];
    Event ev0, ev1;
    uint64_t feat_epoch = 0;
    bool ready() const { return feat != nullptr; }
};

struct Temporal {
    DevBuf<double> hist[2];
    DevBuf<double> count_in;
    DevBuf<unsigned long long> accepted;
    int cur = -1;
    MfxCamera cam{};
    uint64_t epoch = 0;
    bool ready() const { return accepted != nullptr; }
};

struct KeptScene {
    std::vector<mfx_prim> prims;
    std::vector<double> albedo;
    std::vector<mfx_instance> instances;
    std::vector<mfx_quad_light> lights;
    mfx_scene_desc desc{};
    bool instanced = false;
    bool flatten = false;
    bool gpu_bvh = false;
};

struct Readback {
    HostBuf<uint8_t> stage;
    size_t stage_bytes = 0;
    Event stage_ev[kStageChunks];
    Event band_ev[kStageChunks];
    Stream copy_stream;
};

struct CreateEnv {
    using Int = std::optional<int>;
    bool node_f32 = false, diag_iter = false, no_gray_light = false, no_lit_in_hit = false;
    Int mega_waves, shadow_target_blocks, stack_lds, ntop, slot_lds, shadow_waves, blocks_per_cu, camera_packets, cam_blocks;
    Int camera_cuts, camera_cut_cap, camera_cut_min_samples;
    Int pool_fail_once, adaptive_check, iter_events, queue_from, qchunk, ray_queue, mega_chunk, shd_half, chunk;
    std::optional<int64_t> pool;
};

struct CamCuts {
    bool on = true;
    int cap = MFX_CUT_CAP_DEFAULT;
    int min_samples = MFX_CUT_MIN_SAMPLES;
    DevBuf<MfxCutEntry> table;
    DevBuf<MfxCutStats> stats;
    size_t entries = 0;
    bool valid = false;
    MfxCamera cam{};
    uint64_t image_gen = 0;
    int64_t builds = 0;
    Event e0, e1;
    MfxCutStats last{};
    bool last_read = false;
    float last_ms = 0.f;
};

struct Multi {
    bool device_list = false;
    std::vector<std::unique_ptr<mfx_ctx>> peers;
    std::vector<ncclComm_t> comms;
    DevBuf<double> merge;
    bool accum_merged = true;
    DevBuf<double> reduce_stage;
    std::vector<Event> peer_done;
    Event reduce_done;
    bool any() const { return !peers.empty() || !comms.empty(); }
};

}

struct __attribute__((visibility("hidden"))) mfx_ctx {
    int device = 0;
    mfxh::Stream stream;
    MfxHostScene host;
    mfxh::DevBuf<MfxNode> d_nodes;
    mfxh::DevBuf<MfxSlot> d_slots;
    mfxh::DevBuf<MfxNodeH> d_nodes_h;
    mfxh::DevBuf<int32_t> d_slot_ref;
    mfxh::DevBuf<uint8_t> d_ref_blob;
    mfxh::DevBuf<MfxShade> d_shade;
    mfxh::DevBuf<MfxInstance> d_inst;
    double* d_accum = nullptr;
    mfxh::DevBuf<double> d_accum_own;
    mfxh::DevBuf<double> d_film;
    mfxh::DevBuf<double> d_frame;
    mfxh::DevBuf<uint8_t> d_rgba;
    mfxh::DevBuf<unsigned long long> d_work;
    mfxh::DevBuf<unsigned long long> d_counters;
    mfxh::DevBuf<unsigned long long> d_counters_total;
    mfxh::HostBuf<unsigned long long> h_counters;
    uint64_t seed = 0;
    int flags = 0;
    int part_index = 0, part_count = 1;
    int api_part_count = 1;
    int band_index = 0, band_count = 1;
    int64_t next_sample = 0;
    double frame_count = 0.0;
    uint64_t cam_epoch = 0;
    int64_t cam_rebuilds = 0;
    uint64_t image_gen = 0;
    mfxh::CamCuts cuts;
    mfxh::KeptScene kept;
    int grid = 0;
    int stack_size = 1;
    int64_t npix = 0;
    mfxh::Event ev0, ev1;
    bool ev_valid = false;
    std::vector<mfxh::Event> it_ev;
    int it_recorded = 0;
    int it_per_gen = 0;
    int generations = 0;
    bool mega_last = false;
    bool cam_last = false;
    int wf_ext_grid = 0, wf_shd_grid = 0;
    int wf_cam_grid = 0;
    int wf_chunk = 256;
    bool wf_shd_half = true;
    int mega_chunk = 0;
    int mega_waves = 1;
    mfxh::DevBuf<int32_t> d_spill;
    int spill_deep = 0, spill_lanes = 0;
    mfxh::DevBuf<double> d_vscratch;
    mfxh::DevBuf<double> d_albedo;
    mfxh::DevBuf<MfxLight> d_light;
    mfxh::DevBuf<MfxLight> d_lights;
    mfxh::DevBuf<MfxCamera> d_cam;
    mfxh::DevBuf<const void*> d_refs;
    bool rep_valid = false;
    double rep_counts[16] = {0};
    double rep_timing[8] = {0};
    double rep_ms = 0.0;
    mfxh::CreateEnv env;
    bool diag_iter = false;
    bool iter_events = true;
    mfxh::WfPool pool;
    mfxh::Ahead ahead;
    mfxh::Adaptive adp;
    mfxh::Denoise dn;
    mfxh::Temporal tp;
    mfxh::Readback rb;
    mfxh::Multi multi;

    ~mfx_ctx();
};

namespace mfxh __attribute__((visibility("hidden"))) {

inline std::vector<mfx_ctx*> devs_of(mfx_ctx* c) {
    std::vector<mfx_ctx*> v{c};
    for (const auto& p : c->multi.peers) v.push_back(p.get());
    return v;
}

inline int band_rows(const mfx_ctx* d) {
    const int tr = (d->host.height + 7) / 8;
    return band_row_count(d->band_index, d->band_count, tr);
}

inline bool wf_multi_light(const mfx_ctx* c) { return c->host.lights.size() >= 2; }

inline size_t pool_slot_bytes(const mfx_ctx* c) {
    const int nv = c->host.max_depth + 1;
    return WF_DOUBLES_PER_SLOT(nv) * 8 + WF_WORDS_PER_SLOT(nv) * 4 + (wf_multi_light(c) ? WF_LIGHT_BYTES_PER_SLOT(nv) : 0);
}

template <typename P>
void fill_scene_ptrs(const mfx_ctx* c, P& p) {
    p.nodes = c->d_nodes;
    p.slots = c->d_slots;
    p.slot_ref = c->d_slot_ref;
    p.ref_blob = c->d_ref_blob;
    p.shade = c->d_shade;
    p.inst = c->d_inst;
    p.tslack = c->host.tslack;
}

inline bool wf_gray_light(const mfx_ctx* c) {
    const double* I = c->host.light.color;
    return std::memcmp(&I[0], &I[1], sizeof(double)) == 0 && std::memcmp(&I[0], &I[2], sizeof(double)) == 0 &&
           !c->env.no_gray_light && !wf_multi_light(c);
}
inline bool wf_lit_in_hit(const mfx_ctx* c) {
    return c->host.max_depth <= 3 && c->host.shade.size() <= ((size_t)1 << 25) && !c->env.no_lit_in_hit;
}

int whole_film_single_device(const mfx_ctx* c, const char* who);

int wf_trace(mfx_ctx* c, int64_t ns, int64_t sample_base, TraceMode mode = {});
bool cuts_apply(const mfx_ctx* c);
int cuts_ensure(mfx_ctx* c);
int cuts_read_stats(mfx_ctx* c);
int dev_trace_accumulate(mfx_ctx* c, int32_t spp, int64_t sample_base, ResolveSplit* split = nullptr);
int settle_queue_auto(mfx_ctx* c);
void note_live(mfx_ctx* c, const unsigned long long* h);
void sum_counters(const unsigned long long* h, double out[16]);
int add_stage_times(mfx_ctx* c, double out[8]);
int reduce_planes(mfx_ctx* c, double* (*buf)(mfx_ctx*), double* dst, const char* what);
int host_readback(mfx_ctx* c, void* dst, const void* src, size_t bytes, hipStream_t st);
int ahead_materialize(mfx_ctx* c);
int ahead_break(mfx_ctx* c);

}
```

mafrixraytracing_amd/csrc/mfx_trace.cpp:

```cpp
#include "mfx_build.h"
#include "mfx_ctx.h"

using namespace mfxh;

static int wf_ensure_pool(mfx_ctx* c, int32_t pool, bool queues) {
    WfPool& wp = c->pool;
    if (pool <= wp.slots && (!queues || wp.queues)) return MFX_OK;
    const size_t P = (size_t)pool;
    const int nv = c->host.max_depth + 1;
    const size_t per_slot = pool_slot_bytes(c) - (queues ? 0 : WF_QUEUE_BYTES_PER_SLOT);
    const size_t bytes = P * per_slot + 64 * 256;
    size_t mfree = 0, mtotal = 0, headroom = 0;
    if (hipMemGetInfo(&mfree, &mtotal) == hipSuccess && mfree > 0) {
        const size_t avail = mfree + (wp.mem ? wp.bytes : 0);
        headroom = std::min<size_t>((size_t)2 << 30, avail / 4);
        if (bytes + headroom > avail)
            return fail(MFX_E_NOMEM, "wavefront pool: " + std::to_string(bytes >> 20) + " MiB with " +
                                         std::to_string(avail >> 20) + " MiB free");
    }
    wp.mem.reset();
    wp.slots = 0;
    wp.bytes = 0;
    const hipError_t e = wp.mem.alloc(wp.fail_once ? ((size_t)1 << 50) : bytes);
    wp.fail_once = false;
    if (e != hipSuccess) {
        (void)hipGetLastError();
        return fail(e == hipErrorOutOfMemory ? MFX_E_NOMEM : MFX_E_DEVICE,
                    std::string("wavefront pool: ") + hipGetErrorString(e));
    }
    if (headroom > 0 && hipMemGetInfo(&mfree, &mtotal) == hipSuccess && mfree < headroom) {
        wp.mem.reset();
        return fail(MFX_E_NOMEM, "wavefront pool: " + std::to_string(bytes >> 20) + " MiB left " +
                                     std::to_string(mfree >> 20) + " MiB free");
    }
    wp.bytes = bytes;
    char* p = wp.mem;
    auto take = [&](size_t n) { char* r = p; p += (n + 255) & ~(size_t)255; return r; };
    WfParams& A = wp.params;
    double** dbl[6] = {&A.ox, &A.oy, &A.oz, &A.dx, &A.dy, &A.dz};
    for (double** d : dbl) *d = (double*)take(P * 8);
    A.vei = (double*)take(P * 8 * nv);
    A.vls = (double*)take(P * 8 * 2 * nv);
    A.vmat = (WfMat*)take(P * sizeof(WfMat) * nv);
    A.vlt = wf_multi_light(c) ? (uint8_t*)take(P * WF_LIGHT_BYTES_PER_SLOT(nv)) : nullptr;
    A.vstride = (int64_t)P;
    A.rn = (uint32_t*)take(P * 4);
    A.depth = (int32_t*)take(P * 4);
    A.state = (int32_t*)take(P * 4);
#if MFX_RAY_QUEUE
    if (queues) {
        WfQueue& q0 = wp.wq[0];
        double** q0d[6] = {&q0.ox, &q0.oy, &q0.oz, &q0.dx, &q0.dy, &q0.dz};
        for (double** d : q0d) *d = (double*)take(P * 8);
        q0.rn = (uint32_t*)take(P * 4);
        WfQueue& q1 = wp.wq[1];
        q1.ox = A.ox; q1.oy = A.oy; q1.oz = A.oz;
        q1.dx = A.dx; q1.dy = A.dy; q1.dz = A.dz;
        q1.rn = A.rn;
        for (WfQueue* q : {&q0, &q1}) {
            q->depth = (int32_t*)take(P * 4);
            q->state = (int32_t*)take(P * 4);
            q->slot = (int32_t*)take(P * 4);
        }
        q0.count = wp.ctl;
        q1.count = wp.ctl - WF_CTL_Q0 + WF_CTL_Q1;
    }
#endif
    wp.slots = pool;
    wp.queues = queues;
    return MFX_OK;
}

static void wf_queue_views(mfx_ctx* c, WfParams& P, int d) {
    const WfParams& A = c->pool.params;
    P.ox = A.ox; P.oy = A.oy; P.oz = A.oz; P.dx = A.dx; P.dy = A.dy; P.dz = A.dz;
    P.rn = A.rn; P.depth = A.depth; P.state = A.state;
    P.fstate = A.state;
    P.qslot = nullptr;
    P.qcount = nullptr;
    P.ncount = nullptr;
    const int q = c->pool.queue_start();
    if (q < 0 || d < 0) return;
    if (d > q) {
        const WfQueue& R = c->pool.wq[(d - q - 1) & 1];
        P.ox = R.ox; P.oy = R.oy; P.oz = R.oz; P.dx = R.dx; P.dy = R.dy; P.dz = R.dz;
        P.rn = R.rn; P.depth = R.depth; P.state = R.state;
        P.qslot = R.slot;
        P.qcount = R.count;
    }
    if (d >= q && d < P.max_depth) {
        const WfQueue& N = c->pool.wq[(d - q) & 1];
        P.nox = N.ox; P.noy = N.oy; P.noz = N.oz; P.ndx = N.dx; P.ndy = N.dy; P.ndz = N.dz;
        P.nrn = N.rn; P.ndepth = N.depth; P.nstate = N.state; P.nslot = N.slot;
        P.ncount = N.count;
    }
}

template <typename P>
static void fill_trace_params(mfx_ctx* c, P& p, int64_t sample_base) {
    fill_scene_ptrs(c, p);
    p.light = c->host.light;
    p.cam = c->host.camera;
    p.accum = c->d_accum;
    c->adp.accum_valid = false;
    p.seed = c->seed;
    p.sample_base = sample_base;
    p.part_index = c->part_index;
    p.part_count = c->part_count;
    p.band_index = c->band_index;
    p.band_count = c->band_count;
    p.band_rows = band_rows(c);
    p.width = c->host.width;
    p.height = c->host.height;
    p.max_depth = c->host.max_depth;
    p.stack_size = c->stack_size;
}

static void fill_scene_params(mfx_ctx* c, WfParams& P) {
#if MFX_NODE_F16
    P.nodes_h = c->d_nodes_h;
#endif
    P.light_dev = c->d_light;
    P.lights = wf_multi_light(c) ? c->d_lights.get() : nullptr;
    P.nlights = wf_multi_light(c) ? (int32_t)c->host.lights.size() : 0;
    P.cam_dev = c->d_cam;
    P.refs_dev = c->d_refs;
    P.gray_light = wf_gray_light(c);
    P.lit_in_hit = wf_lit_in_hit(c);
    P.albedo = c->d_albedo;
    P.nmat = (int32_t)(c->host.albedo.size() / 3);
}

bool mfxh::cuts_apply(const mfx_ctx* c) { return c->host.inst.empty() && c->wf_cam_grid > 0 && c->cuts.on; }

int mfxh::cuts_ensure(mfx_ctx* c) {
    CamCuts& K = c->cuts;
    if (K.valid && K.image_gen == c->image_gen && std::memcmp(&K.cam, &c->host.camera, sizeof(MfxCamera)) == 0) return MFX_OK;
    const size_t tiles = (size_t)((c->host.width + 7) / 8) * (size_t)((c->host.height + 7) / 8);
    if (K.entries < tiles * K.cap) {
        HIP_TRY(K.table.alloc(tiles * K.cap), _e == hipErrorOutOfMemory ? MFX_E_NOMEM : MFX_E_DEVICE, "camera cuts: ");
        K.entries = tiles * K.cap;
    }
    if (!K.stats) {
        HIPCHECK(K.stats.alloc(1));
        HIPCHECK(K.e0.create());
        HIPCHECK(K.e1.create());
    }
    K.valid = false;
    HIPCHECK(hipEventRecord(K.e0, c->stream));
    HIPCHECK(mfx_build_cut_table(c->d_nodes, c->d_cam, c->host.width, c->host.height, K.cap, K.table, K.stats, c->stream));
    HIPCHECK(hipEventRecord(K.e1, c->stream));
    K.cam = c->host.camera;
    K.image_gen = c->image_gen;
    K.valid = true;
    K.builds += 1;
    K.last_read = false;
    return MFX_OK;
}

int mfxh::cuts_read_stats(mfx_ctx* c) {
    CamCuts& K = c->cuts;
    if (K.builds == 0 || K.last_read) return MFX_OK;
    HIPCHECK(hipSetDevice(c->device));
    HIPCHECK(hipEventSynchronize(K.e1));
    HIPCHECK(hipEventElapsedTime(&K.last_ms, K.e0, K.e1));
    HIPCHECK(hipMemcpy(&K.last, K.stats, sizeof(MfxCutStats), hipMemcpyDeviceToHost));
    K.last_read = true;
    return MFX_OK;
}

int mfxh::wf_trace(mfx_ctx* c, int64_t ns, int64_t sample_base, TraceMode mode) {
    const FrameMode* fm = std::get_if<FrameMode>(&mode);
    ResolveSplit* split = std::holds_alternative<ResolveSplit*>(mode) ? std::get<ResolveSplit*>(mode) : nullptr;
    const TileList* list = std::get_if<TileList>(&mode);
    WfPool& wp = c->pool;
    const int W = c->host.width, H = c->host.height;
    const int brows = band_rows(c);
    if (list && (list->ntiles < 1 || !list->tiles || !list->mom)) return fail(MFX_E_INVALID, "wf_trace: bad tile list");
    const int64_t per_sample = list ? (int64_t)list->ntiles * 64 : (int64_t)((W + 7) / 8) * brows * 64;
    const int64_t total = per_sample * ns;
    if (total == 0) return fail(MFX_E_STATE, "wf_trace: empty band");
    const int qf = wp.queue_start();
    int64_t gen_max = 0;
    int32_t pool = 0;
    int rc = MFX_OK;
    int64_t cap = wp.cap > 0 ? wp.cap : wp.max;
    if (cap < wp.max) {
        const double full = (double)std::min<int64_t>(total, wp.max) * pool_slot_bytes(c);
        size_t mfree = 0, mtotal = 0;
        if (hipMemGetInfo(&mfree, &mtotal) == hipSuccess && 2.0 * full < (double)(mfree + wp.bytes))
            cap = wp.max;
    }
    while (true) {
        const int64_t gcap = list ? std::min(cap, list->gen_paths) : cap;
        gen_max = std::min<int64_t>(total, std::max<int64_t>(4096, gcap / 4096 * 4096));
        pool = (int32_t)((gen_max + 4095) / 4096 * 4096);
        rc = wf_ensure_pool(c, pool, qf >= 0);
        if (rc != MFX_E_NOMEM || cap <= (1 << 20)) break;
        cap = std::max<int64_t>(1 << 20, gen_max / 2);
    }
    if (rc) return rc;
    wp.cap = cap < wp.max ? cap : 0;
    WfParams P = wp.params;
    fill_trace_params(c, P, sample_base);
    fill_scene_params(c, P);
    P.ctl = wp.ctl - WF_CTL_Q0;
    P.counters = fm ? fm->counters : c->d_counters.get();
    const bool own_events = fm == nullptr;
    const bool iter_events = own_events && c->iter_events;
    P.ninst_lds = std::min<int>((int)c->host.inst.size(), WF_INST_LDS);
    P.spill = c->d_spill;
    P.chunk = c->wf_chunk;
    P.tile_padding = (W % 8 != 0 || H % 8 != 0 || (list && list->tile_n)) ? 1 : 0;
    const int32_t chunk0 = P.chunk;
    P.film = fm ? fm->film : nullptr;
    P.frames = fm ? fm->frames : nullptr;
    P.count0 = fm ? fm->count0 : 0.0;
    P.tiles = list ? list->tiles : nullptr;
    P.ntiles = list ? list->ntiles : 0;
    P.mom = list ? list->mom : nullptr;
    P.tile_n = list ? list->tile_n : nullptr;
    P.list_max = list ? list->list_max : 0;
    const bool stats = (c->flags & MFX_F_COUNT_STATS) != 0;
    P.cam_grid = c->host.inst.empty() ? c->wf_cam_grid : 0;
    if (own_events) c->cam_last = P.cam_grid > 0;
    P.cuts = nullptr;
    P.cut_cap = 0;
    if (P.cam_grid > 0 && cuts_apply(c)) {
        const CamCuts& K = c->cuts;
        const bool have = K.valid && K.image_gen == c->image_gen && std::memcmp(&K.cam, &c->host.camera, sizeof(MfxCamera)) == 0;
        if (have || ns >= K.min_samples) {
            MFX_TRY(cuts_ensure(c));
            P.cuts = K.table;
            P.cut_cap = K.cap;
        }
    }
    const int64_t ngen = (total + gen_max - 1) / gen_max;
    const int per_gen = P.max_depth + 1;
    const int iters = (int)ngen * per_gen;
    while (iter_events && (int)c->it_ev.size() < 3 * iters) {
        Event e;
        HIPCHECK(e.create());
        c->it_ev.push_back(std::move(e));
    }
    auto diag = [&](int64_t g, const char* what, int d, float fe, float fs) -> int {
        HIPCHECK(hipStreamSynchronize(c->stream));
        unsigned long long h[WF_NCTR * WF_SHARDS];
        HIPCHECK(hipMemcpy(h, c->d_counters, sizeof(h), hipMemcpyDeviceToHost));
        double r[WF_NCTR] = {0};
        for (int k = 0; k < WF_SHARDS; ++k)
            for (int q = 0; q < WF_NCTR; ++q) r[q] += (double)h[WF_NCTR * k + q];
        for (int q = WF_CTR_ITER + 1; q < WF_CTR_ITER + WF_ITER_CTRS; ++q) r[1] += r[q];
        fprintf(stderr, "gen %lld %s %d: cumulative primary %.0f ext %.0f shadow %.0f; extend %.3f ms shadow %.3f ms;"
                " stamps %.4g %.4g %.4g %.4g outer %.4g node %.4g; cumulative traversal closest %.0f %.0f %.0f"
                " shadow %.0f %.0f %.0f; scan %.4g shade %.4g lat %.4g\n", (long long)g, what, d,
                r[0], r[1], r[2], fe, fs, r[10], r[11], r[12], r[13], r[14], r[15], r[4], r[5], r[6], r[7], r[8], r[9],
                r[16], r[17], r[3]);
        return MFX_OK;
    };
    HIPCHECK(hipEventRecord(fm ? fm->e0 : c->ev0.get(), c->stream));
    int it = 0;
    for (int64_t g = 0; g < ngen; ++g) {
        P.path_base = g * gen_max;
        P.base_smp = P.path_base / per_sample;
        P.base_q = P.path_base % per_sample;
        P.total = std::min<int64_t>(gen_max, total - P.path_base);
        P.pool = (int32_t)((P.total + 4095) / 4096 * 4096);
        HIPCHECK(hipMemsetAsync(P.state, 0, sizeof(int32_t) * (size_t)P.pool, c->stream));
        for (int d = 0; d < per_gen; ++d, ++it) {
            P.start = d == 0 ? 1 : 0;
            P.iter = d;
            wf_queue_views(c, P, d);
            P.chunk = P.qcount ? wp.qchunk : chunk0;
            P.chunk_shd = (c->wf_shd_half && !P.qcount && total <= ((int64_t)1 << 25)) ? std::max(64, P.chunk / 2) : P.chunk;
            if (!iter_events) {
                HIPCHECK(mfx_wf_iteration(P, c->wf_ext_grid, c->wf_shd_grid, stats, c->stream, nullptr));
                continue;
            }
            const Event* ev = c->it_ev.data() + 3 * it;
            hipEvent_t mid = ev[1];
            HIPCHECK(hipEventRecord(ev[0], c->stream));
            HIPCHECK(mfx_wf_iteration(P, c->wf_ext_grid, c->wf_shd_grid, stats, c->stream, &mid));
            HIPCHECK(hipEventRecord(ev[2], c->stream));
            if (c->diag_iter) {
                HIPCHECK(hipStreamSynchronize(c->stream));
                float fe = 0.f, fs = 0.f;
                HIPCHECK(hipEventElapsedTime(&fe, ev[0], ev[1]));
                HIPCHECK(hipEventElapsedTime(&fs, ev[1], ev[2]));
                MFX_TRY(diag(g, "iter", d + 1, fe, fs));
            }
        }
        wf_queue_views(c, P, -1);
        if (split && g == ngen - 1) {
            const int tiles_x = (W + 7) / 8;
            for (int k = 0; k < split->nbands; ++k) {
                const int tx0 = (int)((int64_t)k * tiles_x / split->nbands);
                const int tx1 = (int)((int64_t)(k + 1) * tiles_x / split->nbands);
                P.res_tx0 = tx0;
                P.res_ntx = tx1 - tx0;
                if (P.res_ntx > 0) HIPCHECK(mfx_wf_resolve(P, c->stream));
                MFX_TRY(split->after(k, tx0, tx1 - tx0));
            }
            P.res_tx0 = P.res_ntx = 0;
            split->used = true;
        } else {
            HIPCHECK(mfx_wf_resolve(P, c->stream));
        }
    }
    if (!own_events) {
        HIPCHECK(hipEventRecord(fm->e1, c->stream));
        return MFX_OK;
    }
    HIPCHECK(hipEventRecord(c->ev1, c->stream));
    c->ev_valid = true;
    if (wp.queue_from == -2 && !wp.auto_read) wp.auto_pending = true;
    c->it_recorded = iter_events ? iters : 0;
    c->it_per_gen = per_gen;
    c->generations = (int)ngen;
    return MFX_OK;
}

int mfxh::dev_trace_accumulate(mfx_ctx* c, int32_t spp, int64_t sample_base, ResolveSplit* split) {
    HIPCHECK(hipSetDevice(c->device));
    int64_t ns = spp > c->part_index ? (spp - c->part_index + c->part_count - 1) / c->part_count : 0;
    if (band_rows(c) == 0) ns = 0;
    HIPCHECK(hipMemsetAsync(c->d_work, 0, 64, c->stream));
    HIPCHECK(hipMemsetAsync(c->d_counters, 0, kCounterBytes, c->stream));
    c->mega_last = !wf_multi_light(c) && ((c->flags & MFX_F_MEGAKERNEL) != 0 || (ns == 1 && (c->flags & MFX_F_WAVEFRONT) == 0));
    if (ns == 0) {
        HIPCHECK(hipEventRecord(c->ev0, c->stream));
        HIPCHECK(hipEventRecord(c->ev1, c->stream));
        c->ev_valid = true;
        c->it_recorded = 0;
        c->generations = 0;
        return MFX_OK;
    }
    if (!c->mega_last) {
        MFX_TRY(wf_trace(c, ns, sample_base, split ? TraceMode{split} : TraceMode{}));
        HIPCHECK(mfx_launch_counters_add(c->d_counters_total, c->d_counters, WF_NCTR * WF_SHARDS, c->stream));
        return MFX_OK;
    }
    TraceParams P;
    std::memset(&P, 0, sizeof(P));
    fill_trace_params(c, P, sample_base);
    P.work_counter = c->d_work;
    P.counters = c->d_counters;
    P.nsamples = ns;
    P.vscratch = c->d_vscratch;
    P.waves = c->mega_waves;
    if (c->mega_chunk > 0) {
        P.chunk = c->mega_chunk;
    } else {
        const int64_t total = (int64_t)((c->host.width + 7) / 8) * band_rows(c) * 64 * ns;
        int64_t ch = 256;
        while (ch > 64 && total / ch < 16 * (int64_t)c->grid * 4) ch /= 2;
        P.chunk = (int)ch;
    }
    HIPCHECK(hipEventRecord(c->ev0, c->stream));
    HIPCHECK(mfx_launch_trace(P, (c->flags & MFX_F_COUNT_STATS) != 0, c->grid, c->stream));
    HIPCHECK(hipEventRecord(c->ev1, c->stream));
    c->ev_valid = true;
    HIPCHECK(mfx_launch_counters_add(c->d_counters_total, c->d_counters, WF_NCTR * WF_SHARDS, c->stream));
    return MFX_OK;
}

int mfxh::settle_queue_auto(mfx_ctx* c) {
    for (mfx_ctx* d : devs_of(c)) {
        if (!d->pool.auto_pending) continue;
        HIPCHECK(hipSetDevice(d->device));
        HIPCHECK(hipMemcpyAsync(d->h_counters, d->d_counters, kCounterBytes, hipMemcpyDeviceToHost, d->stream));
        HIPCHECK(hipStreamSynchronize(d->stream));
        note_live(d, d->h_counters);
        d->pool.auto_pending = false;
        d->pool.auto_read = true;
    }
    HIPCHECK(hipSetDevice(c->device));
    return MFX_OK;
}

int mfxh::reduce_planes(mfx_ctx* c, double* (*buf)(mfx_ctx*), double* dst, const char* what) {
    Multi& m = c->multi;
    if (!m.comms.empty()) {
        const Rccl* R = rccl();
        const size_t count = 3 * (size_t)c->npix;
        const std::vector<mfx_ctx*> ds = devs_of(c);
// ... 209 lines not shown
```

mafrixraytracing_amd/csrc/mfx_trace_common.h:

```cpp
#ifndef MFX_TRACE_COMMON_H
#define MFX_TRACE_COMMON_H

#include <hip/hip_runtime.h>
#include <stdint.h>

#include "mfx_camera_cuts.h"
#include "mfx_layout.h"

struct DV {
    double x, y, z;
};
__device__ __forceinline__ DV dv(double x, double y, double z) { return DV{x, y, z}; }
__device__ __forceinline__ DV ld3(const double* p) { return DV{p[0], p[1], p[2]}; }
__device__ __forceinline__ DV vsub(DV a, DV b) { return dv(a.x - b.x, a.y - b.y, a.z - b.z); }
__device__ __forceinline__ DV vadd(DV a, DV b) { return dv(a.x + b.x, a.y + b.y, a.z + b.z); }
__device__ __forceinline__ DV vmul(DV v, double a) { return dv(v.x * a, v.y * a, v.z * a); }
__device__ __forceinline__ DV vdiv(DV v, double a) { return dv(v.x / a, v.y / a, v.z / a); }
__device__ __forceinline__ double vdot(DV a, DV b) { return a.x * b.x + a.y * b.y + a.z * b.z; }
__device__ __forceinline__ DV vcross(DV a, DV v) {
    return dv(a.y * v.z - a.z * v.y, a.z * v.x - a.x * v.z, a.x * v.y - a.y * v.x);
}
__device__ __forceinline__ double vlen(DV v) { return sqrt(v.x * v.x + v.y * v.y + v.z * v.z); }
__device__ __forceinline__ DV vnormalize(DV v) {
    double l = vlen(v);
// ... 789 lines not shown
    const bool pop = nh == 0 && sp > 0;
    const int next = nh > 0 ? c[0] : (pop ? top : MFX_TRAV_EXIT);
    sp += nh > 0 ? nh - 1 : (pop ? -1 : 0);
    return next;
}

__device__ __forceinline__ void cswap3(float& da, int& ca, uint64_t& ma, float& db, int& cb, uint64_t& mb) {
    const bool s = db < da;
    const float t = da;
    const int u = ca;
    const uint64_t w = ma;
    da = s ? db : da;
    ca = s ? cb : ca;
    ma = s ? mb : ma;
    db = s ? t : db;
    cb = s ? u : cb;
    mb = s ? w : mb;
}
struct PacketPlanes {
    int nx, fx, ny, fy, nz, fz;
};

template <bool UNI>
__device__ __forceinline__ int packet_node_step(const MfxNode* __restrict__ nodes, int node, uint64_t& mask,
                                                const RayF& r, float tlim, int* stk, uint64_t* stm, int& sp, int rep,
                                                const PacketPlanes& pp) {
    mfx_cf4* q = (mfx_cf4*)(nodes + node);
    float n[4], f[4];
    const mfx_i4 ch = ((mfx_ci4*)q)[6];
    if (UNI) {
        const mfx_f4 NX = q[pp.nx], FX = q[pp.fx], NY = q[pp.ny], FY = q[pp.fy], NZ = q[pp.nz], FZ = q[pp.fz];
#pragma unroll
        for (int k = 0; k < 4; ++k) {
            const float ax = fmaf(NX[k], r.ix, -r.oix), bx = fmaf(FX[k], r.ix, -r.oix);
            const float ay = fmaf(NY[k], r.iy, -r.oiy), by = fmaf(FY[k], r.iy, -r.oiy);
            const float az = fmaf(NZ[k], r.iz, -r.oiz), bz = fmaf(FZ[k], r.iz, -r.oiz);
            n[k] = fmaxf(fmaxf(ax, ay), fmaxf(az, 0.0f));
            f[k] = fminf(fminf(bx, by), fminf(bz, tlim));
        }
    } else {
        const mfx_f4 lx = q[0], hx = q[1], ly = q[2], hy = q[3], lz = q[4], hz = q[5];
        Slab4 SL;
        slab4(float4{lx.x, lx.y, lx.z, lx.w}, float4{hx.x, hx.y, hx.z, hx.w}, float4{ly.x, ly.y, ly.z, ly.w},
              float4{hy.x, hy.y, hy.z, hy.w}, float4{lz.x, lz.y, lz.z, lz.w}, float4{hz.x, hz.y, hz.z, hz.w}, r, SL);
#pragma unroll
        for (int k = 0; k < 4; ++k) {
            const float a0 = SL.a0[k], a1 = SL.a1[k], b0 = SL.b0[k], b1 = SL.b1[k], c0 = SL.c0[k], c1 = SL.c1[k];
            n[k] = fmaxf(fmaxf(fminf(a0, a1), fminf(b0, b1)), fmaxf(fminf(c0, c1), 0.0f));
            f[k] = fminf(fminf(fmaxf(a0, a1), fmaxf(b0, b1)), fminf(fmaxf(c0, c1), tlim));
        }
    }
    int c[4] = {ch.x, ch.y, ch.z, ch.w};
    uint64_t m[4];
    int nh = 0;
    float d[4];
#pragma unroll
    for (int k = 0; k < 4; ++k) {
        m[k] = __builtin_amdgcn_ballot_w64(n[k] <= f[k]) & mask;
        const bool h = __builtin_amdgcn_inverse_ballot_w64(m[k]);
        const float kd = __int_as_float(__builtin_amdgcn_readlane(__float_as_int(h ? n[k] : 3.0e38f), rep));
        d[k] = m[k] ? kd : __builtin_inff();
        nh += m[k] ? 1 : 0;
    }
    cswap3(d[0], c[0], m[0], d[1], c[1], m[1]);
    cswap3(d[2], c[2], m[2], d[3], c[3], m[3]);
    cswap3(d[0], c[0], m[0], d[2], c[2], m[2]);
    cswap3(d[1], c[1], m[1], d[3], c[3], m[3]);
    cswap3(d[1], c[1], m[1], d[2], c[2], m[2]);
    nh = __builtin_amdgcn_readfirstlane(nh);
    if (__lane_id() == 0) {
        if (nh >= 2) {
            stk[sp] = nh == 4 ? c[3] : (nh == 3 ? c[2] : c[1]);
            stm[sp] = nh == 4 ? m[3] : (nh == 3 ? m[2] : m[1]);
        }
        if (nh >= 3) {
            stk[sp + 1] = nh == 4 ? c[2] : c[1];
            stm[sp + 1] = nh == 4 ? m[2] : m[1];
        }
        if (nh >= 4) {
            stk[sp + 2] = c[1];
            stm[sp + 2] = m[1];
        }
    }
    int next;
    if (nh > 0) {
        next = c[0];
        mask = m[0];
        sp += nh - 1;
    } else if (sp > 0) {
        --sp;
        next = stk[sp];
        mask = stm[sp];
    } else {
        next = MFX_TRAV_EXIT;
    }
    mask = ((uint64_t)__builtin_amdgcn_readfirstlane((int)(mask >> 32)) << 32) |
           (uint32_t)__builtin_amdgcn_readfirstlane((int)(uint32_t)mask);
    return __builtin_amdgcn_readfirstlane(next);
}

template <bool STATS, bool PH, bool UNI>
__device__ __forceinline__ void packet_walk_from(const SceneView& S, DV o, DV d, const RayF& rf, int node, uint64_t mask,
                                                 const int rep, const double tMax, float& tlim, Best& B, int* stk,
                                                 uint64_t* stm, Stats& st, uint32_t& pk_nodes, uint32_t& pk_slots,
                                                 uint64_t* ph, const PacketPlanes& pp) {
    int sp = 0;
    uint64_t t0 = 0;
    while (true) {
        if (PH) t0 = diag_clock();
        while (node >= 0) {
            if (STATS && ((mask >> __lane_id()) & 1)) st.nodes++;
            if (STATS) pk_nodes++;
            if (PH) ph[2]++;
            node = packet_node_step<UNI>(S.nodes, node, mask, rf, tlim, stk, stm, sp, rep, pp);
        }
        if (PH) {
            const uint64_t t1 = diag_clock();
            ph[0] += t1 - t0;
            t0 = t1;
        }
        if (node == MFX_TRAV_EXIT) return;
        if (STATS) pk_slots += (~node & 7) + 1;
        if ((mask >> __lane_id()) & 1) {
            leaf_hit<false, STATS, true>(S, ~node, o, d, 1e-6, tMax, B, st);
            tlim = f_tlim(B.t);
        }
        if (PH) {
            ph[1] += diag_clock() - t0;
            ph[3]++;
        }
        if (sp > 0) {
            --sp;
            node = __builtin_amdgcn_readfirstlane(stk[sp]);
            const uint64_t mm = stm[sp];
            mask = ((uint64_t)__builtin_amdgcn_readfirstlane((int)(mm >> 32)) << 32) |
                   (uint32_t)__builtin_amdgcn_readfirstlane((int)(uint32_t)mm);
        } else {
            return;
        }
    }
}
template <bool STATS, bool PH, bool UNI>
__device__ __forceinline__ void packet_walk(const SceneView& S, DV o, DV d, const RayF& rf, uint64_t mask, Best& B,
                                            int* stk, uint64_t* stm, Stats& st, uint32_t& pk_nodes,
                                            uint32_t& pk_slots, uint64_t* ph, const PacketPlanes& pp) {
    const double tMax = B.t;
    float tlim = f_tlim(tMax);
    packet_walk_from<STATS, PH, UNI>(S, o, d, rf, 0, mask, __builtin_ctzll(mask), tMax, tlim, B, stk, stm, st, pk_nodes,
                                     pk_slots, ph, pp);
}
#ifndef MFX_CUT_LB_CULL
#define MFX_CUT_LB_CULL 1
#endif
template <bool STATS, bool PH, bool UNI>
__device__ __forceinline__ void packet_walk_cuts(const SceneView& S, DV o, DV d, const RayF& rf, const uint64_t mask, Best& B,
                                                 int* stk, uint64_t* stm, Stats& st, uint32_t& pk_nodes,
                                                 uint32_t& pk_slots, uint32_t& pk_cuts, uint64_t* ph,
                                                 const PacketPlanes& pp, const MfxCutEntry* __restrict__ row, const int cap) {
    const double tMax = B.t;
    float tlim = f_tlim(tMax);
    const int rep = __builtin_ctzll(mask);
    mfx_ci4* q = (mfx_ci4*)row;
    mfx_i4 e0 = q[0], e1 = q[1];
    for (int i = 0; i < cap; ++i) {
        const int code = e0.x;
        if (code == MFX_CUT_END) break;
        const float lb = __int_as_float(e0.y);
        const float lox = __int_as_float(e0.z), loy = __int_as_float(e0.w), loz = __int_as_float(e1.x);
        const float hix = __int_as_float(e1.y), hiy = __int_as_float(e1.z), hiz = __int_as_float(e1.w);
        if (i + 1 < cap) {
            e0 = q[2 * i + 2];
            e1 = q[2 * i + 3];
        }
        if (STATS) pk_cuts++;
        if (MFX_CUT_LB_CULL && (__builtin_amdgcn_ballot_w64(lb <= tlim) & mask) == 0) break;
        uint64_t m = mask;
        if (code != 0) {
            const float a0 = fmaf(lox, rf.ix, -rf.oix), a1 = fmaf(hix, rf.ix, -rf.oix);
            const float b0 = fmaf(loy, rf.iy, -rf.oiy), b1 = fmaf(hiy, rf.iy, -rf.oiy);
            const float c0 = fmaf(loz, rf.iz, -rf.oiz), c1 = fmaf(hiz, rf.iz, -rf.oiz);
            const float n = fmaxf(fmaxf(fminf(a0, a1), fminf(b0, b1)), fmaxf(fminf(c0, c1), 0.0f));
            const float f = fminf(fminf(fmaxf(a0, a1), fmaxf(b0, b1)), fminf(fmaxf(c0, c1), tlim));
            m = __builtin_amdgcn_ballot_w64(n <= f) & mask;
            if (m == 0) continue;
        }
        packet_walk_from<STATS, PH, UNI>(S, o, d, rf, code, m, rep, tMax, tlim, B, stk, stm, st, pk_nodes, pk_slots, ph, pp);
    }
}
template <bool STATS, bool PH = false, bool CUTS = false>
__device__ __forceinline__ void packet_closest(const SceneView& S, bool act, DV o, DV d, double tMax, Best& B,
                                               int* stk, uint64_t* stm, Stats& st, uint32_t& pk_nodes,
                                               uint32_t& pk_slots, uint64_t* ph = nullptr,
                                               const MfxCutEntry* row = nullptr, int cap = 0, uint32_t* pk_cuts = nullptr) {
    B = Best{tMax, -1, -1, false};
    const RayF rf = make_rayf(o, d);
    const uint64_t mask = __ballot(act);
    if (mask == 0) return;
    const uint64_t nx = __ballot(act && rf.ix < 0.0f), ny = __ballot(act && rf.iy < 0.0f),
                   nz = __ballot(act && rf.iz < 0.0f);
    const bool uni = (nx == 0 || nx == mask) && (ny == 0 || ny == mask) && (nz == 0 || nz == mask);
    if (uni) {
        const int sx = nx ? 1 : 0, sy = ny ? 1 : 0, sz = nz ? 1 : 0;
        const PacketPlanes pp{sx, 1 - sx, 2 + sy, 3 - sy, 4 + sz, 5 - sz};
        if constexpr (CUTS) packet_walk_cuts<STATS, PH, true>(S, o, d, rf, mask, B, stk, stm, st, pk_nodes, pk_slots, *pk_cuts, ph, pp, row, cap);
        else packet_walk<STATS, PH, true>(S, o, d, rf, mask, B, stk, stm, st, pk_nodes, pk_slots, ph, pp);
    } else {
        const PacketPlanes pp{0, 1, 2, 3, 4, 5};
        if constexpr (CUTS) packet_walk_cuts<STATS, PH, false>(S, o, d, rf, mask, B, stk, stm, st, pk_nodes, pk_slots, *pk_cuts, ph, pp, row, cap);
        else packet_walk<STATS, PH, false>(S, o, d, rf, mask, B, stk, stm, st, pk_nodes, pk_slots, ph, pp);
    }
}

template <bool SHADOW, bool STATS, bool INST = false>
__device__ bool traverse(const SceneView& S, DV o, DV d, double tMin, double tMax, int* __restrict__ stack,
                         Best& B, Stats& st) {
    B = Best{tMax, -1, -1, false};
    RayF rf = make_rayf(o, d);
    float tlim = f_tlim(tMax + S.tslack);
    int sp = 0;
    int node = 0;
    int inst = -1, inst_sp = 0;
    const LdsStack stk{stack};
    while (true) {
        while (node >= 0) {
            if (STATS) st.nodes++;
            node = node_step<false, SHADOW>(S.nodes, node, rf, tlim, stk, sp);
            if (INST) node = inst_frame(S, node, inst, inst_sp, sp, o, d, rf);
        }
        if (node == MFX_TRAV_EXIT) return B.found;
        const int base = (INST && inst >= 0) ? load_inst(S, inst).slot_base : 0;
        const bool better = leaf_hit<SHADOW, STATS>(S, ~node, o, d, tMin, tMax, B, st, base);
        if (better) {
            if (SHADOW) {
                B.found = true;
                return true;
            }
            tlim = f_tlim(B.t);
        }
        if (sp == 0) return B.found;
        node = stack[(--sp) * 64];
        if (INST) node = inst_frame(S, node, inst, inst_sp, sp, o, d, rf);
    }
}

static constexpr double INVPI = 1. / 3.141592653589793;
static constexpr double TWOPI = 2. * 3.141592653589793;

#endif
```

mafrixraytracing_amd/csrc/mfx_wavefront.hip:

```cpp
#include <hip/hip_runtime.h>
#include <stdint.h>

#include <algorithm>
#include <type_traits>
#include <utility>

#include "mfx_device.h"
#include "mfx_trace_common.h"
#include "mfx_wavefront.h"

#ifndef MFX_TRAV_WAVES
#define MFX_TRAV_WAVES 4
#endif

__device__ __forceinline__ int lane_id() { return threadIdx.x & 63; }


#ifndef MFX_SHADOW_ORDER
#define MFX_SHADOW_ORDER 1
#endif

#ifndef MFX_NODE_LANES_MIN
#define MFX_NODE_LANES_MIN 16
#endif
// ... 452 lines not shown
            const double v = ((double)y + rng_next(key, rn)) / (double)P.height;
            const MfxCamera& CAM = P.cam;
            const DV target = vadd(vadd(ld3(CAM.topleft), vmul(ld3(CAM.right), u)), vmul(ld3(CAM.down), v));
            o = ld3(CAM.position);
            d = vnormalize(vsub(target, o));
        } else {
            o = dv(P.ox[s], P.oy[s], P.oz[s]);
            d = dv(P.dx[s], P.dy[s], P.dz[s]);
        }
        trav_begin(T, S, o, d, 99999999.);
        active = true;
    };
    auto finish_ray = [&]() {
        const int s = se & WF_ENTRY_SLOT;
        const bool fresh = START && se < 0;
        const int fl = fresh ? WF_FRESH : 0;
        if (T.B.found) {
            const DV hp = vadd(T.o, vmul(T.d, T.B.t));
            P.ox[s] = hp.x; P.oy[s] = hp.y; P.oz[s] = hp.z;
            const int lm = (P.lit_in_hit && lit_in_entry && !fresh) ? ((se >> 28) & 7) << 29 : 0;
            P.state[s] = ((T.B.info & MFX_INFO_SHADE_MASK) << WF_SHADE_SHIFT) | WF_HIT | fl | lm;
        } else {
            const int lm = fresh || Q ? 0 : (lit_in_entry ? (se >> 28) & 7 : (P.depth[s] >> WF_LIT_SHIFT) & 0xffff);
            P.state[s] = WF_MISS | (lm << WF_SHADE_SHIFT) | fl;
        }
        active = false;
    };

    while (true) {
        bool idle = !active;
        uint64_t m = __ballot(idle);
        while (m != 0) {
            if (pend_lo == pend_hi) {
                int n = 0;
                while (n < 64 && sc.window(P.ctl + WF_CTL_EXT, P.chunk, shard_size, P.state, Q ? P.qcount : nullptr, P.ctl + WF_CTL_CLOSED_EXT)) {
                    if (DG) dg.windows++;
                    const int j = sc.win_next + lane;
                    const int sj = sc.word();
                    bool take = (sj & WF_STATE_MASK) == WF_NEED_EXT;
                    if (START && sj == WF_FREE && j < P.total) {
                        int x, y;
                        int64_t smp;
                        take = !P.tile_padding || path_pixel<LIST>(P, P.path_base + j, x, y, smp);
                    }
                    const uint64_t tm = __ballot(take);
                    if (take)
                        pend[n + __popcll(tm & lanes_below())] =
                            (START && sj == WF_FREE) ? (j | (int)0x80000000)
                                          : (lit_in_entry ? j | (((unsigned)sj >> WF_SHADE_SHIFT) & 7) << 28 : j);
                    n += __popcll(tm);
                    sc.advance(P.state);
                }
                wave_lds_sync();
                pend_lo = 0;
                pend_hi = n;
                c_listed += (uint32_t)n;
                if (n == 0) break;
            }
            const int avail = pend_hi - pend_lo;
            const int rank = __popcll(m & lanes_below());
            if (idle && rank < avail) {
                start_ray(pend[pend_lo + rank]);
                idle = false;
            }
            const int pm = __popcll(m);
            pend_lo += pm < avail ? pm : avail;
            m = __ballot(idle);
        }
        if (!__any(active)) break;
        DIAG_MARK(dg, fetch, DG);
        if (DG) dg.outer++;
        bool fin = false;
        if (active) fin = trav_step<false, STATS, INST, SLDS, NF>(T, S, stack, tn, st, dg, DG);
        DIAG_MARK(dg, leaf, DG);
        if (fin) finish_ray();
        DIAG_MARK(dg, fin, DG);
    }
    unsigned long long* cnt = P.counters + WF_NCTR * (blockIdx.x & (WF_SHARDS - 1));
    const uint32_t c_wave = lane == 0 ? c_listed : 0u;
    block_add<4>(cnt + 0, P.start ? c_wave : 0u, red);
    block_add<4>(cnt + (P.iter > 0 && P.iter < WF_ITER_CTRS ? WF_CTR_ITER + P.iter : 1), P.start ? 0u : c_wave, red);
    if (DG) block_add<4>(cnt + 15, dg.node_iters, red);
    if (DG && lane == 0) {
        atomicAdd(cnt + 10, (unsigned long long)dg.fetch);
        atomicAdd(cnt + 11, (unsigned long long)dg.node);
        atomicAdd(cnt + 12, (unsigned long long)dg.leaf);
        atomicAdd(cnt + 13, (unsigned long long)dg.fin);
        atomicAdd(cnt + 14, (unsigned long long)dg.outer);
        atomicAdd(cnt + 3, (unsigned long long)dg.lat);
    }
    if (STATS) {
        block_add<4>(cnt + 4, st.nodes, red);
        block_add<4>(cnt + 5, st.clusters, red);
        block_add<4>(cnt + 6, st.prims, red);
#ifdef MFX_DIAG_OCCLUSION
        block_add<4>(cnt + 13, st.after_nodes, red);
        block_add<4>(cnt + 14, st.after_leaves, red);
#endif
    }
}

#ifndef MFX_CAM_WAVES
#define MFX_CAM_WAVES 5
#endif
template <bool STATS, int LIST = WF_LIST_NONE, bool CUTS = false>
__global__ void __launch_bounds__(256, MFX_CAM_WAVES) k_camera(WfParams P) {
    extern __shared__ int lds_all[];
    const int lane = lane_id();
    const int wave = threadIdx.x >> 6;
    uint64_t* stm = (uint64_t*)lds_all + wave * P.stack_size;
    int* stk = (int*)((uint64_t*)lds_all + 4 * P.stack_size) + wave * P.stack_size;
    uint32_t* red = (uint32_t*)((int*)((uint64_t*)lds_all + 4 * P.stack_size) + 4 * P.stack_size);
    MfxCamera* cam_lds = (MfxCamera*)(red + 16);
    if (threadIdx.x < sizeof(MfxCamera) / 8) ((double*)cam_lds)[threadIdx.x] = ((const double*)P.cam_dev)[threadIdx.x];
    SceneRefs* refs_lds = (SceneRefs*)(cam_lds + 1);
    if (threadIdx.x == 64) *refs_lds = SceneRefs{(const int32_t*)P.refs_dev[0], (const uint8_t*)P.refs_dev[1]};
    __syncthreads();
    const SceneView S{P.nodes, P.slots, nullptr, nullptr, P.inst, nullptr, 0, nullptr, 0, refs_lds};
    const int shard_size = P.pool / WF_SHARDS;
    Scanner sc{};
    sc.shard = blockIdx.x & (WF_SHARDS - 1);
    uint32_t c_primary = 0;
    Stats st{0, 0, 0};
    uint32_t pk_nodes = 0, pk_slots = 0;
    uint32_t pk_cuts = 0;
#if MFX_DIAG_STAMPS == 3
    uint64_t ph[4] = {0, 0, 0, 0}, t_scan = 0, t_gen = 0, t_out = 0, t_last = stamp();
#define CAM_MARK(acc)                  \
    do {                               \
        const uint64_t _t = stamp();   \
        (acc) += _t - t_last;          \
        t_last = _t;                   \
    } while (0)
#else
#define CAM_MARK(acc) \
    do {              \
    } while (0)
#endif
    while (sc.window<false>(P.ctl + WF_CTL_EXT, P.chunk, shard_size, P.state, nullptr, P.ctl + WF_CTL_CLOSED_EXT)) {
        const int jw = __builtin_amdgcn_readfirstlane(sc.win_next);
        sc.win_next += 64;
        const int j = jw + lane;
        int x = 0, y = 0;
        int64_t smp = 0;
        path_pixel<LIST>(P, P.path_base + jw, x, y, smp);
        const MfxCutEntry* row = nullptr;
        if (CUTS)
            row = P.cuts + (size_t)__builtin_amdgcn_readfirstlane((y >> 3) * ((P.width + 7) >> 3) + (x >> 3)) * (size_t)P.cut_cap;
        x += lane & 7;
        y += lane >> 3;
        const bool act = j < P.total && x < P.width && y < P.height;
        if (!__any(act)) continue;
        CAM_MARK(t_scan);
        DV o = dv(0, 0, 0), d = dv(0, 0, 1);
        if (act) {
            const int64_t pixel = (int64_t)x * P.height + y;
            const int64_t gsample = path_gsample<LIST>(P, smp);
            const uint64_t key = path_key(P.seed, (uint64_t)pixel, (uint64_t)gsample);
            uint32_t rn = 0;
            const double u = ((double)x + rng_next(key, rn)) / (double)P.width;
            const double v = ((double)y + rng_next(key, rn)) / (double)P.height;
            const MfxCamera& CAM = *cam_lds;
            const DV target = vadd(vadd(ld3(CAM.topleft), vmul(ld3(CAM.right), u)), vmul(ld3(CAM.down), v));
            o = ld3(CAM.position);
            d = vnormalize(vsub(target, o));
            c_primary++;
        }
        Best B;
#if MFX_DIAG_STAMPS == 3
        CAM_MARK(t_gen);
        packet_closest<STATS, true, CUTS>(S, act, o, d, 99999999., B, stk, stm, st, pk_nodes, pk_slots, ph, row, P.cut_cap, &pk_cuts);
        t_last = stamp();
#else
        packet_closest<STATS, false, CUTS>(S, act, o, d, 99999999., B, stk, stm, st, pk_nodes, pk_slots, nullptr, row, P.cut_cap,
                                           &pk_cuts);
#endif
        if (act) {
            if (B.found) {
                const DV hp = vadd(o, vmul(d, B.t));
                P.ox[j] = hp.x; P.oy[j] = hp.y; P.oz[j] = hp.z;
                P.state[j] = ((B.info & MFX_INFO_SHADE_MASK) << WF_SHADE_SHIFT) | WF_HIT | WF_FRESH;
            } else {
                P.state[j] = WF_MISS | WF_FRESH;
            }
        }
        CAM_MARK(t_out);
    }
#undef CAM_MARK
    unsigned long long* cnt = P.counters + WF_NCTR * (blockIdx.x & (WF_SHARDS - 1));
    block_add<4>(cnt + 0, c_primary, red);
#if MFX_DIAG_STAMPS == 3
    if (lane == 0) {
        atomicAdd(cnt + 10, (unsigned long long)t_scan);
        atomicAdd(cnt + 11, (unsigned long long)t_gen);
        atomicAdd(cnt + 12, (unsigned long long)ph[0]);
        atomicAdd(cnt + 13, (unsigned long long)ph[1]);
        atomicAdd(cnt + 14, (unsigned long long)t_out);
        atomicAdd(cnt + 15, (unsigned long long)ph[2]);
        atomicAdd(cnt + 16, (unsigned long long)ph[3]);
    }
#endif
    if (STATS) {
        block_add<4>(cnt + 4, st.nodes, red);
        block_add<4>(cnt + 5, st.clusters, red);
        block_add<4>(cnt + 6, st.prims, red);
        block_add<4>(cnt + 10, lane == 0 ? pk_nodes : 0u, red);
        block_add<4>(cnt + 11, lane == 0 ? pk_slots : 0u, red);
#if MFX_DIAG_STAMPS != 3
        if (CUTS) block_add<4>(cnt + 12, lane == 0 ? pk_cuts : 0u, red);
#endif
    }
}

struct PixParams {
    int64_t path_base, base_q, base_smp, sample_base;
    uint64_t seed;
    int32_t width, height;
    union {
        struct { int32_t band_index, band_count; };
        const int32_t* tiles;
    };
    union {
        struct { int32_t band_rows, part_index; };
        const int32_t* tile_n;
    };
    union {
        int32_t part_count;
        int32_t list_max;
    };
    int32_t ntiles;
};
static_assert(sizeof(PixParams) == 72, "PixParams: k_shadow's LDS layout");
struct ShdPtrs {
    double *ox, *oy, *oz, *dx, *dy, *dz, *vei, *vls;
    WfMat* vmat;
    uint32_t* rn;
    int32_t* depth;
    const MfxShade* shade;
    int32_t* fstate;
    const int32_t* qslot;
    double *nox, *noy, *noz, *ndx, *ndy, *ndz;
    uint32_t* nrn;
    int32_t *ndepth, *nstate, *nslot;
    unsigned long long* ncount;
    unsigned long long *ctl, *counters;
    int32_t* state;
    const unsigned long long* qcount;
};

template <bool STATS, bool SPILL, int WAVES, int SK, bool Q, int LIST = WF_LIST_NONE, int NF = MFX_NF_ANY, bool ML = false>
__global__ void __launch_bounds__(256, WAVES) k_shadow(WfParams P) {
    constexpr bool INST = SK == WF_SK_INST, SLDS = SK == WF_SK_SLDS;
    extern __shared__ int lds_all[];
#if MFX_NODE_F16
    const TopNodes tn{(const float4*)lds_all, P.ntop_shd, P.nodes_h};
#else
    const TopNodes tn{(const float4*)lds_all, P.ntop_shd};
#endif
    MfxInstance* inst_lds = (MfxInstance*)(lds_all + P.ntop_shd * 32);
    int4* slot_lds = (int4*)(inst_lds + (INST ? P.ninst_lds : 0));
    const int nslot = SLDS ? P.nslot_shd : 0;
    int* lds = (int*)(slot_lds + 5 * nslot);
    uint8_t* pend_base = (uint8_t*)(lds + 4 * P.stack_lds_shd * 64);
    uint32_t* red = (uint32_t*)(pend_base + 4 * PendShd::BYTES);
    MfxLight* light_lds = (MfxLight*)((int*)(red + 16) + 4 * 2 * WF_SHD_LIST);
    if constexpr (ML) {
        if (threadIdx.x == 3) *(MlPtrs*)light_lds = MlPtrs{P.lights, P.vlt, P.nlights};
    } else {
        if (threadIdx.x < sizeof(MfxLight) / 8)
            ((double*)light_lds)[threadIdx.x] = ((const double*)P.light_dev)[threadIdx.x];
    }
    if (threadIdx.x == 0)
        *(ShdPtrs*)(light_lds + 1) = ShdPtrs{P.ox, P.oy, P.oz, P.dx, P.dy, P.dz, P.vei, P.vls, P.vmat, P.rn, P.depth,
                                            P.shade, P.fstate, P.qslot, P.nox, P.noy, P.noz, P.ndx, P.ndy, P.ndz,
                                            P.nrn, P.ndepth, P.nstate, P.nslot, P.ncount, P.ctl, P.counters, P.state,
                                            P.qcount};
    SceneRefs* refs_lds = (SceneRefs*)((PixParams*)((ShdPtrs*)(light_lds + 1) + 1) + 1);
    if (threadIdx.x == 2)
        *refs_lds = SceneRefs{(const int32_t*)P.refs_dev[0], (const uint8_t*)P.refs_dev[1]};
    if (threadIdx.x == 1) {
        PixParams px;
        px.path_base = P.path_base; px.base_q = P.base_q; px.base_smp = P.base_smp; px.sample_base = P.sample_base;
        px.seed = P.seed; px.width = P.width; px.height = P.height;
        if (LIST) {
            px.tiles = P.tiles;
        } else {
            px.band_index = P.band_index; px.band_count = P.band_count;
        }
        if (LIST == WF_LIST_TILE_N) {
            px.tile_n = P.tile_n; px.list_max = P.list_max;
        } else {
            px.band_rows = P.band_rows; px.part_index = P.part_index; px.part_count = P.part_count;
        }
        px.ntiles = LIST ? P.ntiles : 0;
        *(PixParams*)((ShdPtrs*)(light_lds + 1) + 1) = px;
    }
#if MFX_NODE_F16
    if (NF == MFX_NF_H || (NF == MFX_NF_ANY && P.nodes_h)) load_top_nodes_h((float4*)lds_all, P.nodes_h, P.ntop_shd);
    else
#endif
        load_top_nodes((float4*)lds_all, P.nodes, P.ntop_shd);
    if (INST) load_inst_lds(inst_lds, P.inst, P.ninst_lds);
    if (SLDS) load_slots_lds(slot_lds, P.slots, nslot);
    const MfxLight& LT = *light_lds;
    [[maybe_unused]] const MlPtrs& M = *(const MlPtrs*)light_lds;
    const ShdPtrs& C = *(const ShdPtrs*)(light_lds + 1);
    const PixParams& PX = *(const PixParams*)((const ShdPtrs*)(light_lds + 1) + 1);
    const int lane = lane_id();
    const int wave = threadIdx.x >> 6;
    using Stack = typename std::conditional<SPILL, SpillStack, LdsStack>::type;
    const Stack stack = make_stack<SPILL>(lds + wave * P.stack_lds_shd * 64 + lane, P, P.stack_lds_shd);
    const PendShd pd(pend_base + wave * PendShd::BYTES);
    const SceneView S{P.nodes, P.slots, nullptr, nullptr, P.inst, inst_lds, INST ? P.ninst_lds : 0, slot_lds, nslot, refs_lds, P.tslack};
    const int shard_size = P.pool / WF_SHARDS;

    int* shl = (int*)(red + 16) + wave * 2 * WF_SHD_LIST;
    Scanner sc{};
    sc.shard = blockIdx.x & (WF_SHARDS - 1);
    int nshade = 0;
    int pend_lo = 0, pend_hi = 0;
    bool active = false;
    int s = 0;
    Trav T{};
    double scs = 0.0, ssolid = 0.0;
    int vflag = 0;
    uint32_t c_shadow = 0;
    Stats st{0, 0, 0};
// ... 723 lines not shown
```

mafrixraytracing_amd/native.py:

```python
from __future__ import annotations

import ctypes as C

import numpy as np

from .abi import (INSTANCING_KEYS, LAUNCH_INFO_KEYS, MFX_DN_SRC_ACCUM, MFX_DN_SRC_ADAPTIVE, MFX_DN_SRC_HOST,
                  MFX_DN_SRC_TEMPORAL, MFX_F_NONE, MFX_F_TWO_LEVEL, MfxAdaptive, MfxAdaptiveResume, MfxDenoiseCfg,
                  MfxDenoiseVarCfg, MfxInstance, MfxOptions, MfxTemporalCfg, SceneArrays, check, dptr, iptr, load_library,
                  pinhole_struct, quad_lights)
from .denoise import DenoiseConfig, DenoiseVarConfig
from .temporal import TemporalConfig

DEFAULT_SEED = 0x4D414652
DEFAULT_RENDER_AHEAD = 64


class NativeContext:

    def __init__(self, arrays: SceneArrays, seed: int = DEFAULT_SEED, device: int = 0, flags: int = MFX_F_NONE,
                 part_index: int = 0, part_count: int = 1, devices: list[int] | None = None,
                 instancing: bool = True, render_ahead: int = 0, lights: list | None = None):
        self.lib = load_library()
        self.arrays = arrays
        self.w, self.h = arrays.width, arrays.height
# ... 138 lines not shown
                "eps_needed": float(out[14]), "rebuilds": int(out[15])}

    def temporal(self, frame: np.ndarray | None = None, variance: np.ndarray | None = None,
                 count: np.ndarray | None = None, cfg: TemporalConfig | None = None, restart: bool = False,
                 want_rgba: bool = False, **tolerances):
        cfg = cfg if cfg is not None else TemporalConfig(**tolerances)
        c = MfxTemporalCfg(source=MFX_DN_SRC_ADAPTIVE if frame is None else MFX_DN_SRC_HOST, restart=1 if restart else 0,
                           tol_depth=cfg.tol_depth, tol_normal2=cfg.tol_normal2, max_history=cfg.max_history)
        n = self.w * self.h
        src = var = cnt = None
        if frame is not None:
            src = np.ascontiguousarray(frame, dtype=np.float64)
            assert src.size == n * 4
        if variance is not None:
            var = np.ascontiguousarray(variance, dtype=np.float64)
            assert var.size == n
        if count is not None:
            cnt = np.ascontiguousarray(count, dtype=np.float64)
            assert cnt.size == n
        out = np.empty((n, 4), dtype=np.float64)
        vout = np.empty(n, dtype=np.float64)
        nout = np.empty(n, dtype=np.float64)
        rgba = np.empty(n * 4, dtype=np.uint8) if want_rgba else None
        acc = C.c_int64(-1)
        ms = C.c_double()
        check(self.lib.mfx_temporal(self._h, C.byref(c), dptr(src) if src is not None else None,
                                    dptr(var) if var is not None else None, dptr(cnt) if cnt is not None else None,
                                    dptr(out), dptr(vout), dptr(nout),
                                    rgba.ctypes.data_as(C.POINTER(C.c_uint8)) if want_rgba else None, C.byref(acc),
                                    C.byref(ms)), "mfx_temporal")
        self.last_temporal_ms = ms.value
        return (out, vout, nout, acc.value) + ((rgba,) if want_rgba else ())

    def render_rgba8(self, spp: int = 1, want_pixels: bool = True, out: np.ndarray | None = None) -> np.ndarray | None:
        if not want_pixels:
            check(self.lib.mfx_render_rgba8(self._h, spp, None), "mfx_render_rgba8")
            return None
        if out is None:
            out = np.empty(self.w * self.h * 4, dtype=np.uint8)
        assert out.dtype == np.uint8 and out.size == self.w * self.h * 4 and out.flags.c_contiguous
        check(self.lib.mfx_render_rgba8(self._h, spp, out.ctypes.data_as(C.POINTER(C.c_uint8))), "mfx_render_rgba8")
        return out

    def reset(self):
        check(self.lib.mfx_reset(self._h), "mfx_reset")

    def film_mean(self) -> np.ndarray:
        frame = np.empty((self.w * self.h, 4), dtype=np.float64)
        check(self.lib.mfx_film_mean(self._h, dptr(frame)), "mfx_film_mean")
        return frame

    def trace_accumulate(self, spp: int, sample_base: int):
        check(self.lib.mfx_trace_accumulate(self._h, spp, sample_base), "mfx_trace_accumulate")

    def accum_reduce(self):
        check(self.lib.mfx_accum_reduce(self._h), "mfx_accum_reduce")

    def accum_clear(self):
        check(self.lib.mfx_accum_clear(self._h), "mfx_accum_clear")

    def accum_device_ptr(self) -> tuple[int, int]:
        p = C.c_void_p()
        n = C.c_int64()
        check(self.lib.mfx_accum_device_ptr(self._h, C.byref(p), C.byref(n)), "mfx_accum_device_ptr")
        return p.value, n.value

    def accum_attach(self, dptr: int | None, nbytes: int = 0):
        check(self.lib.mfx_accum_attach(self._h, C.c_void_p(dptr) if dptr else None, nbytes), "mfx_accum_attach")

    def accum_read_mean(self, count: float) -> np.ndarray:
        frame = np.empty((self.w * self.h, 4), dtype=np.float64)
        check(self.lib.mfx_accum_read_mean(self._h, float(count), dptr(frame)), "mfx_accum_read_mean")
        return frame

    def sync(self):
        check(self.lib.mfx_sync(self._h), "mfx_sync")

    def stream(self) -> int:
        s = C.c_void_p()
        check(self.lib.mfx_stream(self._h, C.byref(s)), "mfx_stream")
        return s.value or 0

    def ray_counts(self) -> np.ndarray:
        out = np.zeros(16)
        check(self.lib.mfx_ray_counts(self._h, dptr(out)), "mfx_ray_counts")
        return out

    def ray_counts_total(self, reset: bool = True) -> np.ndarray:
        out = np.zeros(16)
        check(self.lib.mfx_ray_counts_total(self._h, dptr(out), 1 if reset else 0), "mfx_ray_counts_total")
        return out

    def stats(self) -> tuple[float, float]:
        rays, sec = C.c_double(), C.c_double()
        check(self.lib.mfx_stats(self._h, C.byref(rays), C.byref(sec)), "mfx_stats")
        return rays.value, sec.value

    def last_trace_ms(self) -> float:
        ms = C.c_double()
        check(self.lib.mfx_last_trace_ms(self._h, C.byref(ms)), "mfx_last_trace_ms")
        return ms.value

    def trace_timing(self) -> dict:
        out = np.zeros(8)
        check(self.lib.mfx_trace_timing(self._h, dptr(out)), "mfx_trace_timing")
        return {"total_ms": out[0], "camera_ms": out[1], "extend_ms": out[2], "camera_launches": int(out[3]),
                "shadow_ms": out[4], "iterations": int(out[5]), "launches": int(out[6]), "generations": int(out[7])}

    def closest_hit(self, rays: np.ndarray, tmin: float = 1e-6, tmax: float = 99999999.0):
        rays = np.ascontiguousarray(rays, dtype=np.float64).reshape(-1, 6)
        n = len(rays)
        t = np.zeros(n)
        prim = np.zeros(n, dtype=np.int32)
        nrm = np.zeros((n, 3))
        check(self.lib.mfx_closest_hit(self._h, n, dptr(rays), tmin, tmax, dptr(t), iptr(prim), dptr(nrm)),
              "mfx_closest_hit")
        return t, prim, nrm

    def any_hit(self, rays: np.ndarray, tmax: np.ndarray, tmin: float = 1e-6):
        rays = np.ascontiguousarray(rays, dtype=np.float64).reshape(-1, 6)
        tmax = np.ascontiguousarray(tmax, dtype=np.float64)
        occ = np.zeros(len(rays), dtype=np.int32)
        check(self.lib.mfx_any_hit(self._h, len(rays), dptr(rays), tmin, dptr(tmax), iptr(occ)), "mfx_any_hit")
        return occ

    def build_info(self) -> dict:
        out = np.zeros(8)
        dig = C.c_uint64()
        check(self.lib.mfx_build_info(self._h, dptr(out), C.byref(dig)), "mfx_build_info")
        return {"ref_bvh_ms": out[0], "bvh_ms": out[1], "scene_ms": out[2], "gpu_bvh": bool(out[3]),
                "gpu_images": bool(out[3] == 2),
                "nodes4": int(out[4]), "slots": int(out[5]), "nodes2": int(out[6]), "levels": int(out[7]),
                "digest": dig.value}

    def device_info(self) -> dict:
        out = np.zeros(5 + len(self.devices), dtype=np.int32)
        check(self.lib.mfx_device_info(self._h, iptr(out), len(out)), "mfx_device_info")
        g = int(out[0])
        return {"devices": [int(d) for d in out[5:5 + g]], "communicators": int(out[1]),
                "merge": {0: "none", 1: "rccl_reduce", 2: "ordered_adds"}[int(out[2])],
                "band_index": int(out[3]), "band_count": int(out[4])}

    def launch_info(self) -> dict:
        out = np.zeros(len(LAUNCH_INFO_KEYS), dtype=np.int32)
        check(self.lib.mfx_launch_info(self._h, iptr(out), len(out)), "mfx_launch_info")
        flags = ("spill_ext", "spill_shd", "lit_in_hit", "gray_light", "camera_packets", "shd_half", "camera_cuts")
        return {k: bool(v) if k in flags else int(v) for k, v in zip(LAUNCH_INFO_KEYS, out)}

    def camera_cut_info(self) -> dict:
        out = np.zeros(32)
        check(self.lib.mfx_camera_cut_info(self._h, dptr(out)), "mfx_camera_cut_info")
        return {"builds": int(out[0]), "build_ms": float(out[1]), "len_sum": int(out[2]), "len_max": int(out[3]),
                "root_tiles": int(out[4]), "empty_tiles": int(out[5]), "tiles": int(out[6]), "cap": int(out[7]),
                "hist": [int(v) for v in out[8:25]]}

    def camera_cut_table(self, host: bool = False) -> np.ndarray:
        n = C.c_int64()
        check(self.lib.mfx_camera_cut_table(self._h, None, 0, C.byref(n), int(host)), "mfx_camera_cut_table")
        out = np.zeros(n.value, dtype=np.uint8)
        check(self.lib.mfx_camera_cut_table(self._h, out.ctypes.data_as(C.c_void_p), n.value, C.byref(n), int(host)),
              "mfx_camera_cut_table")
        return out.reshape(-1, self.launch_info()["cut_cap"], 32)

    def light_info(self) -> np.ndarray:
        out = np.zeros(8)
        check(self.lib.mfx_light_info(self._h, dptr(out)), "mfx_light_info")
        return out

    def instancing_info(self) -> dict:
        out = np.zeros(8)
        check(self.lib.mfx_instancing_info(self._h, dptr(out)), "mfx_instancing_info")
        return {k: int(v) for k, v in zip(INSTANCING_KEYS, out)}

    def ref_leaves(self):
        n = len(self.arrays.prims)
        idx = np.zeros(n, dtype=np.int32)
        lf = np.zeros(n, dtype=np.int32)
        lc = np.zeros(n, dtype=np.int32)
        nl = C.c_int32()
        check(self.lib.mfx_ref_leaves(self._h, iptr(idx), iptr(lf), iptr(lc), C.byref(nl)), "mfx_ref_leaves")
        return idx, lf[:nl.value], lc[:nl.value]


def fp64_selftest(a: np.ndarray, b: np.ndarray, device: int = 0):
    lib = load_library()
    a = np.ascontiguousarray(a, dtype=np.float64)
    b = np.ascontiguousarray(b, dtype=np.float64)
    dv = np.zeros_like(a)
    sq = np.zeros_like(a)
    check(lib.mfx_fp64_selftest(device, len(a), dptr(a), dptr(b), dptr(dv), dptr(sq)), "mfx_fp64_selftest")
    return dv, sq


def aabb_selftest(rec: np.ndarray, device: int = 0):
    lib = load_library()
    rec = np.ascontiguousarray(rec, dtype=np.float64).reshape(-1, 24)
    out = np.zeros((len(rec), 3), dtype=np.int32)
    check(lib.mfx_aabb_selftest(device, len(rec), dptr(rec), iptr(out)), "mfx_aabb_selftest")
    return out[:, 0], out[:, 1], out[:, 2]


class Film:

    def __init__(self, ctx: NativeContext):
        self._ctx = ctx
        self.Size = (ctx.w, ctx.h)

    def Reset(self):
        self._ctx.reset()

    def GetFrame(self, integrator: "NativePixelIntegrator", samples: int) -> np.ndarray:
        self._ctx.render_rgba8(samples, want_pixels=False)
        return self._ctx.film_mean()


class NativePixelIntegrator:

    def __init__(self, ctx: NativeContext):
        self._ctx = ctx

    def Sample(self, n: int) -> np.ndarray:
        return self._ctx.sample(n)

    def SampleAdaptive(self, minSpp: int, maxSpp: int, stepSpp: int, relError: float, absFloor: float):
        return self._ctx.sample_adaptive(minSpp, maxSpp, stepSpp, relError, absFloor)

    def SampleAdaptiveResume(self, maxSpp: int, stepSpp: int, maxPasses: int, relError: float, absFloor: float):
        return self._ctx.sample_adaptive_resume(maxSpp, stepSpp, relError, absFloor, max_passes=maxPasses)


class Scene:

    def __init__(self, state, seed: int = DEFAULT_SEED, device: int = 0, max_depth: int = 3,
                 render_ahead: int = DEFAULT_RENDER_AHEAD):
        arrays = state.arrays(max_depth=max_depth) if hasattr(state, "arrays") else state
        self._ctx = NativeContext(arrays, seed=seed, device=device, render_ahead=render_ahead)
        self.width, self.height = arrays.width, arrays.height
        self.film = Film(self._ctx)
        self.pixelIntegrator = NativePixelIntegrator(self._ctx)

    @property
    def ScreenSize(self):
        return (self.width, self.height)

    def Render(self, delta: float, buffer) -> None:
        out = self._ctx.render_rgba8(1)
        mv = memoryview(buffer).cast("B")
        mv[:] = out.tobytes()

    def close(self):
        self._ctx.close()
```

Before: 12560 Mrays/s.

## Cull per-tile camera cut leaf slots and skip primary rays in empty tiles

The camera-cut table builder now runs an exact conservative test on each leaf's slots against the tile frustum. It drops or narrows leaf entries whose slots cannot be hit, and this is enabled once enough samples have accumulated for the camera. Separately, primary rays whose tile has an empty cut skip traversal entirely and are counted as misses. The aim is to cut primary-ray leaf intersection work and traversal for empty tiles. The cost is a more expensive table build, which is deferred behind a sample threshold, plus added correctness checks in the host validator.

```diff
diff --git a/mafrixraytracing_amd/csrc/cut_check.cpp b/mafrixraytracing_amd/csrc/cut_check.cpp
--- a/mafrixraytracing_amd/csrc/cut_check.cpp
+++ b/mafrixraytracing_amd/csrc/cut_check.cpp
@@ -88,6 +88,61 @@
     return v;
 }
 
+std::vector<mfx_prim> adversarial(const mfx_pinhole& def, int W, int H) {
+    MfxCamera cam;
+    mfx_derive_camera(def, cam);
+    std::vector<mfx_prim> v = soup(60, 61);
+    const auto P = [&](double px, double py, double r, double* out) {
+        const mfx_cut::V3 c = mfx_cut::film_dir(cam, px, py, W, H);
+        out[0] = cam.position[0] + r * c.x; out[1] = cam.position[1] + r * c.y; out[2] = cam.position[2] + r * c.z;
+    };
+    const auto tri = [&](const double* a, const double* b, const double* c) {
+        mfx_prim p;
+        std::memset(&p, 0, sizeof(p));
+        p.kind = MFX_PRIM_TRIANGLE;
+        p.material = (int)(v.size() % 3);
+        std::memcpy(p.p[0], a, 24); std::memcpy(p.p[1], b, 24); std::memcpy(p.p[2], c, 24);
+        v.push_back(p);
+    };
+    const int tiles_x = (W + 7) / 8, tiles_y = (H + 7) / 8;
+    const int picks[3][2] = {{0, 0}, {tiles_x / 2, tiles_y / 2}, {tiles_x - 1, tiles_y - 1}};
+    for (const auto& pk : picks) {
+        const double x0 = pk[0] * 8, y0 = pk[1] * 8, x1 = std::min<double>(x0 + 8, W), y1 = std::min<double>(y0 + 8, H);
+        const double xm = 0.5 * (x0 + x1), ym = 0.5 * (y0 + y1);
+        double a[3], b[3], c[3], d[3];
+        for (const double w : {0.0, 1.0}) {
+            P(x0 - w - 3, y0 - w - 2, 2.0, a); P(x0 - w + 3, y0 - w + 2, 2.0, b); P(x0 - w - 6, y0 - w + 7, 2.0, c);
+            tri(a, b, c);
+            tri(b, a, c);
+        }
+        for (const double w : {0.0, 1.0}) {
+            P(x0 - w, y0 - 5, 2.5, a); P(x0 - w, y1 + 5, 2.5, b);
+            P(x0 - w - 9, ym, 2.5, c); tri(a, b, c);
+            P(x0 - w + 9, ym, 2.5, c); tri(a, b, c);
+        }
+        P(x0 - 4, y0, 3.0, a); P(x1 + 4, y0, 3.0, b); P(xm, y0 - 7, 3.0, c); tri(a, b, c);
+        {
+            mfx_prim p;
+            std::memset(&p, 0, sizeof(p));
+            p.kind = MFX_PRIM_RECT;
+            P(x1, y0, 2.2, a); P(x1 + 6, y0, 2.2, b); P(x1 + 6, y1, 2.2, c); P(x1, y1, 2.2, d);
+            std::memcpy(p.p[0], a, 24); std::memcpy(p.p[1], b, 24); std::memcpy(p.p[2], c, 24); std::memcpy(p.p[3], d, 24);
+            v.push_back(p);
+        }
+        for (const double lift : {0.0, 1e-12, 1e-9, 1e-5}) {
+            P(xm, ym, 1.5, a); P(xm, ym, 3.0, b); P(xm + 4, ym + 1, 2.0, c);
+            c[1] += lift;
+            tri(a, b, c);
+        }
+        for (const double off : {0.0, 1e-9}) {
+            a[0] = cam.position[0] + off; a[1] = cam.position[1]; a[2] = cam.position[2];
+            P(x0 - 2, y0 - 2, 2.0, b); P(x1 + 2, ym, 2.0, c);
+            tri(a, b, c);
+        }
+    }
+    return v;
+}
+
 bool load_prims(const char* path, std::vector<mfx_prim>& v) {
     FILE* f = std::fopen(path, "rb");
     if (!f) return false;
@@ -129,15 +184,80 @@
 
 struct Totals {
     long long rays = 0, leaves = 0, uncovered = 0, lb_above = 0, tiles = 0, root = 0, empty = 0, multi = 0;
+    long long accepted = 0, lost = 0, slots_seen = 0, slots_culled = 0, dropped = 0, narrowed = 0;
 };
 
 int find_entry(const MfxCutEntry* row, int cap, int code) {
-    for (int i = 0; i < cap && row[i].code != MFX_CUT_END; ++i)
+    for (int i = 0; i < cap && row[i].code != MFX_CUT_END; ++i) {
         if (row[i].code == code) return i;
+        if (code < 0 && row[i].code < 0) {
+            const int lc = ~code, ec = ~row[i].code;
+            if ((ec >> 3) >= (lc >> 3) && (ec >> 3) + (ec & 7) <= (lc >> 3) + (lc & 7)) return i;
+        }
+    }
     return -1;
 }
 
-void check_ray(const std::vector<MfxNode>& nodes, const RayF& r, const MfxCutEntry* row, int cap, Totals& t) {
+struct D3 {
+    double x, y, z;
+};
+D3 d3(const double* p) { return {p[0], p[1], p[2]}; }
+D3 vsub(D3 a, D3 b) { return {a.x - b.x, a.y - b.y, a.z - b.z}; }
+double vdot(D3 a, D3 b) { return a.x * b.x + a.y * b.y + a.z * b.z; }
+D3 vcross(D3 a, D3 v) { return {a.y * v.z - a.z * v.y, a.z * v.x - a.x * v.z, a.x * v.y - a.y * v.x}; }
+bool tri_hit64(const MfxSlot& s, D3 o, D3 d, double tMin) {
+    const D3 e1 = d3(s.b), e2 = d3(s.c);
+    const D3 s1 = vcross(d, e2);
+    const double divisor = vdot(s1, e1);
+    if (std::fabs(divisor) < 1e-6) return false;
+    const double inv = 1. / divisor;
+    const D3 dd = vsub(o, d3(s.a));
+    const double b1 = vdot(dd, s1) * inv;
+    if (b1 < 0. || b1 > 1.) return false;
+    const D3 s2 = vcross(dd, e1);
+    const double b2 = vdot(d, s2) * inv;
+    if (b2 < 0. || (b1 + b2) >= 1.) return false;
+    const double t = vdot(e2, s2) * inv;
+    return t > tMin;
+}
+bool sphere_hit64(const MfxSlot& s, D3 o, D3 d, double tMin, double tMax) {
+    const D3 oc = vsub(o, d3(s.a));
+    const double a = 1.;
+    const double b = 2.0 * vdot(oc, d);
+    const double c = vdot(oc, oc) - s.b[0] * s.b[0];
+    const double disc = b * b - 4.0 * a * c;
+    if (disc > 0) {
+        const double rd = std::sqrt(disc);
+        const double q = (b < 0.) ? -0.5 * (b - rd) : -0.5 * (b + rd);
+        const double t0 = q, t1 = c / q;
+        const double tmn = t0 < t1 ? t0 : t1, tmx = t0 > t1 ? t0 : t1;
+        if (tmn >= tMin && tmn < tMax) return true;
+        if (tmx > tMin && tmx < tMax) return true;
+    }
+    return false;
+}
+
+void check_leaf_slots(const std::vector<MfxSlot>& slots, int child, const double* o, const double* d, const MfxCutEntry* row,
+                      int cov, Totals& t) {
+    const int lc = ~child, s0 = lc >> 3, n = (lc & 7) + 1;
+    int k0 = 0, k1 = 0;
+    if (cov >= 0) {
+        const int ec = ~row[cov].code;
+        k0 = ec >> 3;
+        k1 = k0 + (ec & 7) + 1;
+    }
+    for (int k = 0; k < n; ++k) {
+        const MfxSlot& sl = slots[s0 + k];
+        const int kind = (sl.info >> MFX_INFO_KIND_SHIFT) & 3;
+        const bool hit = kind == MFX_KIND_SPHERE ? sphere_hit64(sl, d3(o), d3(d), 1e-6, 99999999.) : tri_hit64(sl, d3(o), d3(d), 1e-6);
+        if (!hit) continue;
+        ++t.accepted;
+        if (s0 + k < k0 || s0 + k >= k1) ++t.lost;
+    }
+}
+
+void check_ray(const std::vector<MfxNode>& nodes, const std::vector<MfxSlot>& slots, const RayF& r, const double* o,
+               const double* d, const MfxCutEntry* row, int cap, Totals& t) {
     struct Item {
         int node, cov;
     };
@@ -151,6 +271,7 @@
             float n = 0.f;
             if (!slab(nd, k, r, n)) continue;
             int cov = it.cov;
+            const bool above = cov < 0;
             if (cov < 0) {
                 cov = find_entry(row, cap, nd.child[k]);
                 if (cov >= 0 && !(row[cov].lb <= n)) ++t.lb_above;
@@ -159,7 +280,8 @@
                 stack.push_back({nd.child[k], cov});
             } else {
                 ++t.leaves;
-                if (cov < 0) ++t.uncovered;
+                if (above) check_leaf_slots(slots, nd.child[k], o, d, row, cov, t);
+                if (cov < 0 && !MFX_CUT_SLOT_CULL) ++t.uncovered;
             }
         }
     }
@@ -170,8 +292,10 @@
     const int tiles_x = (W + 7) / 8, tiles_y = (H + 7) / 8;
     std::vector<MfxCutEntry> table((size_t)tiles_x * tiles_y * cap);
     MfxCutStats st;
-    mfx_cut::table_host(s.nodes.data(), cam, W, H, cap, table.data(), st);
+    mfx_cut::table_host(s.nodes.data(), s.slots.data(), cam, W, H, cap, table.data(), st);
     Totals t;
+    t.slots_seen = (long long)st.slots_seen; t.slots_culled = (long long)st.slots_culled;
+    t.dropped = (long long)st.leaves_dropped; t.narrowed = (long long)st.leaves_narrowed;
     t.tiles = (long long)tiles_x * tiles_y;
     t.root = (long long)st.root_tiles;
     t.empty = (long long)st.empty_tiles;
@@ -193,16 +317,18 @@
                 if (l != 0.0)
                     for (int a = 0; a < 3; ++a) d[a] = d[a] / l;
                 ++t.rays;
-                check_ray(s.nodes, make_rayf(o, d), row, cap, t);
+                check_ray(s.nodes, s.slots, make_rayf(o, d), o, d, row, cap, t);
             }
         }
     std::printf("%s %s %dx%d cap=%d: tiles=%lld root=%lld empty=%lld multi=%lld mean_len=%.3f max_len=%llu rays=%lld leaves=%lld"
-                " uncovered=%lld lb_above=%lld\n",
+                " uncovered=%lld lb_above=%lld accepted=%lld lost=%lld slots_seen=%lld slots_culled=%lld dropped=%lld narrowed=%lld\n",
                 scene, camname, W, H, cap, t.tiles, t.root, t.empty, t.multi, (double)st.len_sum / (double)t.tiles, st.len_max,
-                t.rays, t.leaves, t.uncovered, t.lb_above);
+                t.rays, t.leaves, t.uncovered, t.lb_above, t.accepted, t.lost, t.slots_seen, t.slots_culled, t.dropped, t.narrowed);
     if (root_share) *root_share = (double)t.root / (double)t.tiles;
     all.rays += t.rays; all.leaves += t.leaves; all.uncovered += t.uncovered; all.lb_above += t.lb_above;
     all.tiles += t.tiles; all.root += t.root; all.empty += t.empty; all.multi += t.multi;
+    all.accepted += t.accepted; all.lost += t.lost; all.slots_seen += t.slots_seen; all.slots_culled += t.slots_culled;
+    all.dropped += t.dropped; all.narrowed += t.narrowed;
 }
 
 bool build(const std::vector<mfx_prim>& prims, const mfx_pinhole& cam, MfxHostScene& s) {
@@ -271,7 +397,7 @@
     for (const int cap : {MFX_CUT_CAP_MAX, MFX_CUT_CAP_DEFAULT}) {
         std::vector<MfxCutEntry> table((size_t)tiles * cap);
         MfxCutStats st;
-        mfx_cut::table_host(s.nodes.data(), cam, W, H, cap, table.data(), st);
+        mfx_cut::table_host(s.nodes.data(), s.slots.data(), cam, W, H, cap, table.data(), st);
         long long internal = 0, entries = 0;
         for (const MfxCutEntry& e : table)
             if (e.code != MFX_CUT_END) {
@@ -283,6 +409,10 @@
                     entries ? (double)internal / (double)entries : 0.0);
         for (int n = 0; n <= cap; ++n) std::printf(" %d:%llu", n, st.hist[n]);
         std::printf("\n");
+        std::printf("%dx%d cap=%d slot_cull=%d leaf_entry_slots=%llu culled=%llu culled_share=%.4f entries_dropped=%llu"
+                    " entries_narrowed=%llu\n",
+                    W, H, cap, MFX_CUT_SLOT_CULL, st.slots_seen, st.slots_culled,
+                    st.slots_seen ? (double)st.slots_culled / (double)st.slots_seen : 0.0, st.leaves_dropped, st.leaves_narrowed);
     }
     return 0;
 }
@@ -305,13 +435,25 @@
     }
     Totals all;
     int bad = check_scene("soup_600", soup(600, 600), soup_cam, false, all);
+    bad += check_scene("adv_40x24", adversarial(soup_cam, 40, 24), soup_cam, false, all);
+    bad += check_scene("adv_17x9", adversarial(soup_cam, 17, 9), soup_cam, false, all);
     if (!mesh.empty()) bad += check_scene("mesh", mesh, spot_cam, true, all);
-    std::printf("total: rays=%lld leaves=%lld uncovered=%lld lb_above=%lld tiles=%lld root=%lld empty=%lld multi=%lld\n", all.rays,
-                all.leaves, all.uncovered, all.lb_above, all.tiles, all.root, all.empty, all.multi);
+    std::printf("total: rays=%lld leaves=%lld uncovered=%lld lb_above=%lld tiles=%lld root=%lld empty=%lld multi=%lld accepted=%lld"
+                " lost=%lld slots_seen=%lld slots_culled=%lld dropped=%lld narrowed=%lld\n",
+                all.rays, all.leaves, all.uncovered, all.lb_above, all.tiles, all.root, all.empty, all.multi, all.accepted, all.lost,
+                all.slots_seen, all.slots_culled, all.dropped, all.narrowed);
     if (all.uncovered || all.lb_above) {
         std::printf("FAIL: a reached leaf is not covered, or an entry's lb is above a ray's entry distance\n");
         ++bad;
     }
+    if (all.lost) {
+        std::printf("FAIL: a slot the exact test accepts lies outside its tile's kept ranges\n");
+        ++bad;
+    }
+    if (all.accepted == 0 || (MFX_CUT_SLOT_CULL && (all.slots_culled == 0 || all.dropped == 0 || all.narrowed == 0))) {
+        std::printf("FAIL: vacuous (no slot accepted, or the slot cull culled, dropped or narrowed nothing)\n");
+        ++bad;
+    }
     if (all.empty == 0 || all.multi == 0 || all.leaves == 0) {
         std::printf("FAIL: vacuous (no empty cut, no cut of more than one entry, or no leaf reached)\n");
         ++bad;
diff --git a/mafrixraytracing_amd/csrc/mfx_api.cpp b/mafrixraytracing_amd/csrc/mfx_api.cpp
--- a/mafrixraytracing_amd/csrc/mfx_api.cpp
+++ b/mafrixraytracing_amd/csrc/mfx_api.cpp
@@ -79,6 +79,7 @@
     v.camera_cuts = num("MFX_CAMERA_CUTS");
     v.camera_cut_cap = num("MFX_CAMERA_CUT_CAP");
     v.camera_cut_min_samples = num("MFX_CAMERA_CUT_MIN_SAMPLES");
+    v.camera_cut_cull_min_samples = num("MFX_CAMERA_CUT_CULL_MIN_SAMPLES");
     v.pool_fail_once = num("MFX_POOL_FAIL_ONCE");
     v.adaptive_check = num("MFX_ADAPTIVE_CHECK");
     v.iter_events = num("MFX_ITER_EVENTS");
@@ -201,6 +202,7 @@
             c->cuts.on = env.camera_cuts.value_or(1) != 0;
             c->cuts.cap = std::max(1, std::min(env.camera_cut_cap.value_or(MFX_CUT_CAP_DEFAULT), MFX_CUT_CAP_MAX));
             c->cuts.min_samples = std::max(1, env.camera_cut_min_samples.value_or(MFX_CUT_MIN_SAMPLES));
+            c->cuts.cull_min_samples = std::max(1, env.camera_cut_cull_min_samples.value_or(MFX_CUT_CULL_MIN_SAMPLES));
             CK(mfx_cam_occupancy(c->stack_size, &cb, c->cuts.on));
             if (env.cam_blocks) cb = std::min(cb, std::max(1, *env.cam_blocks));
             c->wf_cam_grid = prop.multiProcessorCount * std::max(1, std::min(cb, 8));
@@ -722,12 +724,12 @@
     if (host) {
         std::vector<MfxCutEntry> t(tiles * c->cuts.cap);
         MfxCutStats st;
-        mfx_cut::table_host(c->host.nodes.data(), c->host.camera, c->host.width, c->host.height, c->cuts.cap, t.data(), st);
+        mfx_cut::table_host(c->host.nodes.data(), c->host.slots.data(), c->host.camera, c->host.width, c->host.height, c->cuts.cap, t.data(), st);
         std::memcpy(out, t.data(), bytes);
         return MFX_OK;
     }
     HIPCHECK(hipSetDevice(c->device));
-    MFX_TRY(cuts_ensure(c));
+    MFX_TRY(cuts_ensure(c, INT64_MAX));
     HIPCHECK(hipMemcpyAsync(out, c->cuts.table, bytes, hipMemcpyDeviceToHost, c->stream));
     HIPCHECK(hipStreamSynchronize(c->stream));
     return MFX_OK;
@@ -748,6 +750,11 @@
     out[6] = (double)((int64_t)((c->host.width + 7) / 8) * ((c->host.height + 7) / 8));
     out[7] = (double)K.cap;
     for (int n = 0; n <= MFX_CUT_CAP_MAX; ++n) out[8 + n] = (double)K.last.hist[n];
+    out[25] = (double)K.last.slots_seen;
+    out[26] = (double)K.last.slots_culled;
+    out[27] = (double)K.last.leaves_dropped;
+    out[28] = (double)K.last.leaves_narrowed;
+    out[29] = K.culled ? 1.0 : 0.0;
     return MFX_OK;
 }
 
diff --git a/mafrixraytracing_amd/csrc/mfx_build.h b/mafrixraytracing_amd/csrc/mfx_build.h
--- a/mafrixraytracing_amd/csrc/mfx_build.h
+++ b/mafrixraytracing_amd/csrc/mfx_build.h
@@ -28,7 +28,7 @@
 hipError_t mfx_gpu_build_images(const float* prim_box, const float* cent, const int32_t* weight, int n, int max_leaf,
                                 float c_isect, const MfxGpuLayoutIn& in, MfxGpuImages& out);
 
-hipError_t mfx_build_cut_table(const MfxNode* nodes, const MfxCamera* cam_dev, int W, int H, int cap, MfxCutEntry* table,
-                               MfxCutStats* stats_dev, hipStream_t st);
+hipError_t mfx_build_cut_table(const MfxNode* nodes, const MfxSlot* slots, const MfxCamera* cam_dev, int W, int H, int cap,
+                               MfxCutEntry* table, MfxCutStats* stats_dev, hipStream_t st);
 
 #endif
diff --git a/mafrixraytracing_amd/csrc/mfx_build.hip b/mafrixraytracing_amd/csrc/mfx_build.hip
--- a/mafrixraytracing_amd/csrc/mfx_build.hip
+++ b/mafrixraytracing_amd/csrc/mfx_build.hip
@@ -655,18 +655,24 @@
     return e;
 }
 
-__global__ void __launch_bounds__(64) k_cut_table(const MfxNode* __restrict__ nodes, const MfxCamera* __restrict__ cam, int W, int H,
-                                                  int tiles_x, int ntiles, int cap, MfxCutEntry* __restrict__ table,
-                                                  MfxCutStats* __restrict__ stats) {
+__global__ void __launch_bounds__(64) k_cut_table(const MfxNode* __restrict__ nodes, const MfxSlot* __restrict__ slots,
+                                                  const MfxCamera* __restrict__ cam, int W, int H, int tiles_x, int ntiles, int cap,
+                                                  MfxCutEntry* __restrict__ table, MfxCutStats* __restrict__ stats) {
     __shared__ MfxCutEntry lists[MFX_CUT_CAP_MAX * 64];
     const int t = blockIdx.x * blockDim.x + threadIdx.x;
     const bool valid = t < ntiles;
     int n = -1;
     bool root = false;
+    unsigned tally[4] = {0, 0, 0, 0};
     if (valid) {
         MfxCutEntry* row = table + (size_t)t * cap;
-        n = mfx_cut::tile_cut(nodes, *cam, W, H, t % tiles_x, t / tiles_x, cap, row, lists + threadIdx.x, 64);
+        n = mfx_cut::tile_cut(nodes, slots, *cam, W, H, t % tiles_x, t / tiles_x, cap, row, lists + threadIdx.x, 64, tally);
         root = n == 1 && row[0].code == 0;
+    }
+    for (int k = 0; k < 4; ++k) {
+        unsigned v = tally[k];
+        for (int off = 32; off > 0; off >>= 1) v += __shfl_xor(v, off);
+        if (threadIdx.x == 0 && v) atomicAdd(&stats->slots_seen + k, (unsigned long long)v);
     }
     int sum = valid ? n : 0, mx = sum;
     for (int off = 32; off > 0; off >>= 1) {
@@ -688,13 +694,13 @@
     }
 }
 
-hipError_t mfx_build_cut_table(const MfxNode* nodes, const MfxCamera* cam_dev, int W, int H, int cap, MfxCutEntry* table,
-                               MfxCutStats* stats_dev, hipStream_t st) {
+hipError_t mfx_build_cut_table(const MfxNode* nodes, const MfxSlot* slots, const MfxCamera* cam_dev, int W, int H, int cap,
+                               MfxCutEntry* table, MfxCutStats* stats_dev, hipStream_t st) {
     const int tiles_x = (W + 7) / 8, ntiles = tiles_x * ((H + 7) / 8);
     if (cap < 1 || cap > MFX_CUT_CAP_MAX || ntiles < 1) return hipErrorInvalidValue;
     const hipError_t e = hipMemsetAsync(stats_dev, 0, sizeof(MfxCutStats), st);
     if (e != hipSuccess) return e;
-    hipLaunchKernelGGL(k_cut_table, dim3((ntiles + 63) / 64), dim3(64), 0, st, nodes, cam_dev, W, H, tiles_x, ntiles, cap, table,
-                       stats_dev);
+    hipLaunchKernelGGL(k_cut_table, dim3((ntiles + 63) / 64), dim3(64), 0, st, nodes, slots, cam_dev, W, H, tiles_x, ntiles, cap,
+                       table, stats_dev);
     return hipGetLastError();
 }
diff --git a/mafrixraytracing_amd/csrc/mfx_camera_cuts.h b/mafrixraytracing_amd/csrc/mfx_camera_cuts.h
--- a/mafrixraytracing_amd/csrc/mfx_camera_cuts.h
+++ b/mafrixraytracing_amd/csrc/mfx_camera_cuts.h
@@ -17,7 +17,12 @@
 #define MFX_CUT_END (-0x7fffffff - 1)
 #define MFX_CUT_MIN_GAP 0x1p-16
 #define MFX_CUT_MARGIN 0x1p-17
+#ifndef MFX_CUT_SLOT_CULL
+#define MFX_CUT_SLOT_CULL 1
+#endif
+#define MFX_CUT_SLOT_MARGIN 0x1p-32
 #define MFX_CUT_MIN_SAMPLES 32
+#define MFX_CUT_CULL_MIN_SAMPLES 128
 
 struct alignas(32) MfxCutEntry {
     int32_t code;
@@ -27,6 +32,7 @@
 
 struct MfxCutStats {
     unsigned long long len_sum, len_max, root_tiles, empty_tiles, hist[MFX_CUT_CAP_MAX + 1];
+    unsigned long long slots_seen, slots_culled, leaves_dropped, leaves_narrowed;
 };
 
 namespace mfx_cut {
@@ -52,6 +58,8 @@
 
 struct Pyramid {
     V3 n[4];
+    V3 c[4];
+    double cl[4];
     V3 pos;
     double mpos;
     bool ok;
@@ -67,6 +75,8 @@
     const V3 c00 = film_dir(cam, x0 - 1, y0 - 1, W, H), c01 = film_dir(cam, x1 + 1, y0 - 1, W, H);
     const V3 c10 = film_dir(cam, x0 - 1, y1 + 1, W, H), c11 = film_dir(cam, x1 + 1, y1 + 1, W, H);
     const V3 mid = add(add(c00, c01), add(c10, c11));
+    P.c[0] = c00; P.c[1] = c01; P.c[2] = c10; P.c[3] = c11;
+    for (int i = 0; i < 4; ++i) P.cl[i] = sqrt(dot(P.c[i], P.c[i]));
     const V3 raw[4] = {cross(c00, c10), cross(c01, c11), cross(c00, c01), cross(c10, c11)};
     for (int k = 0; k < 4; ++k) {
         V3 n = raw[k];
@@ -135,8 +145,52 @@
                        {3.402823466e38f, 3.402823466e38f, 3.402823466e38f}};
 }
 
-MFX_CUT_HD int tile_cut(const MfxNode* nodes, const MfxCamera& cam, int W, int H, int tx, int ty, int cap, MfxCutEntry* row,
-                        MfxCutEntry* list, int stride) {
+MFX_CUT_HD bool slot_culled(const Pyramid& P, const MfxSlot& s) {
+    const V3 e1 = v3(s.b), e2 = v3(s.c), dd = sub(P.pos, v3(s.a));
+    const V3 nd = cross(e2, e1), n1 = cross(e2, dd), n2 = cross(dd, e1);
+    const double E = max2(max2(max2(abs1(e1.x), abs1(e1.y)), abs1(e1.z)), max2(max2(abs1(e2.x), abs1(e2.y)), abs1(e2.z)));
+    const double Q = max2(max2(abs1(dd.x), abs1(dd.y)), abs1(dd.z));
+    const double tn = MFX_CUT_SLOT_MARGIN * ((Q + E) * E), td = MFX_CUT_SLOT_MARGIN * (E * E);
+    if (!(tn > 0x1p-900) || !(td > 0x1p-900) || !finite1(tn)) return false;
+    const double s0 = dot(P.c[0], nd) < 0.0 ? -1.0 : 1.0;
+    bool out0 = true, out1 = true, out2 = true;
+    for (int i = 0; i < 4; ++i) {
+        const double hd = s0 * dot(P.c[i], nd), h1 = s0 * dot(P.c[i], n1), h2 = s0 * dot(P.c[i], n2);
+        const double h0 = (hd - h1) - h2;
+        if (!(hd > td * P.cl[i])) return false;
+        const double m = -(tn * P.cl[i]);
+        out0 = out0 && h0 < m;
+        out1 = out1 && h1 < m;
+        out2 = out2 && h2 < m;
+    }
+    return out0 || out1 || out2;
+}
+
+MFX_CUT_HD int cull_leaf(const Pyramid& P, const MfxSlot* slots, int child, int& seen, int& culled) {
+    const int code = ~child;
+    seen = culled = 0;
+    if (!MFX_CUT_SLOT_CULL || !slots || (code & MFX_INST_FLAG)) return child;
+    const int s0 = code >> 3, n = (code & 7) + 1;
+    int first = n, end = 0;
+    for (int k = 0; k < n;) {
+        const int kind = (slots[s0 + k].info >> MFX_INFO_KIND_SHIFT) & 3;
+        const int w = kind == MFX_KIND_RECT && k + 1 < n ? 2 : 1;
+        bool gone = kind != MFX_KIND_SPHERE && slot_culled(P, slots[s0 + k]);
+        if (kind == MFX_KIND_RECT) gone = gone && w == 2 && slot_culled(P, slots[s0 + k + 1]);
+        if (!gone) {
+            if (k < first) first = k;
+            end = k + w;
+        }
+        k += w;
+    }
+    seen = n;
+    culled = end == 0 ? n : n - (end - first);
+    if (end == 0) return MFX_CUT_END;
+    return ~(((s0 + first) << 3) | (end - first - 1));
+}
+
+MFX_CUT_HD int tile_cut(const MfxNode* nodes, const MfxSlot* slots, const MfxCamera& cam, int W, int H, int tx, int ty, int cap,
+                        MfxCutEntry* row, MfxCutEntry* list, int stride, unsigned* tally = nullptr) {
     cap = cap < 1 ? 1 : (cap > MFX_CUT_CAP_MAX ? MFX_CUT_CAP_MAX : cap);
     int n = 1;
     list[0] = root_entry();
@@ -155,10 +209,16 @@
             const MfxNode& nd = nodes[code];
             int k = 0;
             unsigned keep = 0;
+            int ccode[4] = {0, 0, 0, 0}, cseen[4] = {0, 0, 0, 0}, cgone[4] = {0, 0, 0, 0};
             for (int c = 0; c < 4; ++c) {
                 if (nd.child[c] == MFX_CHILD_EMPTY) continue;
                 const float lo[3] = {nd.lox[c], nd.loy[c], nd.loz[c]}, hi[3] = {nd.hix[c], nd.hiy[c], nd.hiz[c]};
                 if (outside(P, lo, hi)) continue;
+                ccode[c] = nd.child[c];
+                if (nd.child[c] < 0) {
+                    ccode[c] = cull_leaf(P, slots, nd.child[c], cseen[c], cgone[c]);
+                    if (ccode[c] == MFX_CUT_END) continue;
+                }
                 keep |= 1u << c;
                 ++k;
             }
@@ -171,9 +231,15 @@
             list[i * stride] = list[n * stride];
             need = (need & ~((uint64_t)15 << (4 * i))) | (((need >> (4 * n)) & 15) << (4 * i));
             for (int c = 0; c < 4; ++c) {
+                if (tally && cseen[c]) {
+                    tally[0] += (unsigned)cseen[c];
+                    tally[1] += (unsigned)cgone[c];
+                    tally[2] += ccode[c] == MFX_CUT_END;
+                    tally[3] += ccode[c] != MFX_CUT_END && ccode[c] != nd.child[c];
+                }
                 if (!((keep >> c) & 1)) continue;
                 MfxCutEntry e;
-                e.code = nd.child[c];
+                e.code = ccode[c];
                 e.lo[0] = nd.lox[c]; e.lo[1] = nd.loy[c]; e.lo[2] = nd.loz[c];
                 e.hi[0] = nd.hix[c]; e.hi[1] = nd.hiy[c]; e.hi[2] = nd.hiz[c];
                 e.lb = lower_bound(P, e.lo, e.hi);
@@ -196,9 +262,10 @@
     for (int i = 0; i < cap; ++i) row[i] = i < n ? list[i * stride] : MfxCutEntry{MFX_CUT_END, 0.0f, {0.0f, 0.0f, 0.0f}, {0.0f, 0.0f, 0.0f}};
     return n;
 }
-inline int tile_cut(const MfxNode* nodes, const MfxCamera& cam, int W, int H, int tx, int ty, int cap, MfxCutEntry* row) {
+inline int tile_cut(const MfxNode* nodes, const MfxSlot* slots, const MfxCamera& cam, int W, int H, int tx, int ty, int cap,
+                    MfxCutEntry* row, unsigned* tally = nullptr) {
     MfxCutEntry list[MFX_CUT_CAP_MAX];
-    return tile_cut(nodes, cam, W, H, tx, ty, cap, row, list, 1);
+    return tile_cut(nodes, slots, cam, W, H, tx, ty, cap, row, list, 1, tally);
 }
 
 MFX_CUT_HD void count_tile(MfxCutStats& s, int n, const MfxCutEntry* row) {
@@ -209,13 +276,19 @@
     s.hist[n] += 1;
 }
 
-inline void table_host(const MfxNode* nodes, const MfxCamera& cam, int W, int H, int cap, MfxCutEntry* table, MfxCutStats& stats) {
+inline void table_host(const MfxNode* nodes, const MfxSlot* slots, const MfxCamera& cam, int W, int H, int cap, MfxCutEntry* table,
+                       MfxCutStats& stats) {
     const int tiles_x = (W + 7) / 8, tiles_y = (H + 7) / 8;
     stats = MfxCutStats{};
     for (int ty = 0; ty < tiles_y; ++ty)
         for (int tx = 0; tx < tiles_x; ++tx) {
             MfxCutEntry* row = table + (size_t)(ty * tiles_x + tx) * cap;
-            count_tile(stats, tile_cut(nodes, cam, W, H, tx, ty, cap, row), row);
+            unsigned tally[4] = {0, 0, 0, 0};
+            count_tile(stats, tile_cut(nodes, slots, cam, W, H, tx, ty, cap, row, tally), row);
+            stats.slots_seen += tally[0];
+            stats.slots_culled += tally[1];
+            stats.leaves_dropped += tally[2];
+            stats.leaves_narrowed += tally[3];
         }
 }
 
diff --git a/mafrixraytracing_amd/csrc/mfx_ctx.h b/mafrixraytracing_amd/csrc/mfx_ctx.h
--- a/mafrixraytracing_amd/csrc/mfx_ctx.h
+++ b/mafrixraytracing_amd/csrc/mfx_ctx.h
@@ -241,7 +241,7 @@
     using Int = std::optional<int>;
     bool node_f32 = false, diag_iter = false, no_gray_light = false, no_lit_in_hit = false;
     Int mega_waves, shadow_target_blocks, stack_lds, ntop, slot_lds, shadow_waves, blocks_per_cu, camera_packets, cam_blocks;
-    Int camera_cuts, camera_cut_cap, camera_cut_min_samples;
+    Int camera_cuts, camera_cut_cap, camera_cut_min_samples, camera_cut_cull_min_samples;
     Int pool_fail_once, adaptive_check, iter_events, queue_from, qchunk, ray_queue, mega_chunk, shd_half, chunk;
     std::optional<int64_t> pool;
 };
@@ -250,6 +250,9 @@
     bool on = true;
     int cap = MFX_CUT_CAP_DEFAULT;
     int min_samples = MFX_CUT_MIN_SAMPLES;
+    int cull_min_samples = MFX_CUT_CULL_MIN_SAMPLES;
+    int64_t cam_samples = 0;
+    bool culled = false;
     DevBuf<MfxCutEntry> table;
     DevBuf<MfxCutStats> stats;
     size_t entries = 0;
@@ -396,7 +399,7 @@
 
 int wf_trace(mfx_ctx* c, int64_t ns, int64_t sample_base, TraceMode mode = {});
 bool cuts_apply(const mfx_ctx* c);
-int cuts_ensure(mfx_ctx* c);
+int cuts_ensure(mfx_ctx* c, int64_t ns);
 int cuts_read_stats(mfx_ctx* c);
 int dev_trace_accumulate(mfx_ctx* c, int32_t spp, int64_t sample_base, ResolveSplit* split = nullptr);
 int settle_queue_auto(mfx_ctx* c);
diff --git a/mafrixraytracing_amd/csrc/mfx_trace.cpp b/mafrixraytracing_amd/csrc/mfx_trace.cpp
--- a/mafrixraytracing_amd/csrc/mfx_trace.cpp
+++ b/mafrixraytracing_amd/csrc/mfx_trace.cpp
@@ -133,9 +133,13 @@
 
 bool mfxh::cuts_apply(const mfx_ctx* c) { return c->host.inst.empty() && c->wf_cam_grid > 0 && c->cuts.on; }
 
-int mfxh::cuts_ensure(mfx_ctx* c) {
+int mfxh::cuts_ensure(mfx_ctx* c, int64_t ns) {
     CamCuts& K = c->cuts;
-    if (K.valid && K.image_gen == c->image_gen && std::memcmp(&K.cam, &c->host.camera, sizeof(MfxCamera)) == 0) return MFX_OK;
+    const bool same = K.valid && K.image_gen == c->image_gen && std::memcmp(&K.cam, &c->host.camera, sizeof(MfxCamera)) == 0;
+    if (!same) K.cam_samples = 0;
+    K.cam_samples = ns > INT64_MAX - K.cam_samples ? INT64_MAX : K.cam_samples + std::max<int64_t>(ns, 0);
+    const bool cull = K.cam_samples >= K.cull_min_samples;
+    if (same && (K.culled || !cull)) return MFX_OK;
     const size_t tiles = (size_t)((c->host.width + 7) / 8) * (size_t)((c->host.height + 7) / 8);
     if (K.entries < tiles * K.cap) {
         HIP_TRY(K.table.alloc(tiles * K.cap), _e == hipErrorOutOfMemory ? MFX_E_NOMEM : MFX_E_DEVICE, "camera cuts: ");
@@ -148,10 +152,11 @@
     }
     K.valid = false;
     HIPCHECK(hipEventRecord(K.e0, c->stream));
-    HIPCHECK(mfx_build_cut_table(c->d_nodes, c->d_cam, c->host.width, c->host.height, K.cap, K.table, K.stats, c->stream));
+    HIPCHECK(mfx_build_cut_table(c->d_nodes, cull ? (const MfxSlot*)c->d_slots : nullptr, c->d_cam, c->host.width, c->host.height, K.cap, K.table, K.stats, c->stream));
     HIPCHECK(hipEventRecord(K.e1, c->stream));
     K.cam = c->host.camera;
     K.image_gen = c->image_gen;
+    K.culled = cull;
     K.valid = true;
     K.builds += 1;
     K.last_read = false;
@@ -230,7 +235,7 @@
         const CamCuts& K = c->cuts;
         const bool have = K.valid && K.image_gen == c->image_gen && std::memcmp(&K.cam, &c->host.camera, sizeof(MfxCamera)) == 0;
         if (have || ns >= K.min_samples) {
-            MFX_TRY(cuts_ensure(c));
+            MFX_TRY(cuts_ensure(c, ns));
             P.cuts = K.table;
             P.cut_cap = K.cap;
         }
diff --git a/mafrixraytracing_amd/csrc/mfx_trace_common.h b/mafrixraytracing_amd/csrc/mfx_trace_common.h
--- a/mafrixraytracing_amd/csrc/mfx_trace_common.h
+++ b/mafrixraytracing_amd/csrc/mfx_trace_common.h
@@ -965,6 +965,9 @@
 #ifndef MFX_CUT_LB_CULL
 #define MFX_CUT_LB_CULL 1
 #endif
+#ifndef MFX_CUT_EMPTY_SKIP
+#define MFX_CUT_EMPTY_SKIP 1
+#endif
 template <bool STATS, bool PH, bool UNI>
 __device__ __forceinline__ void packet_walk_cuts(const SceneView& S, DV o, DV d, const RayF& rf, const uint64_t mask, Best& B,
                                                  int* stk, uint64_t* stm, Stats& st, uint32_t& pk_nodes,
diff --git a/mafrixraytracing_amd/csrc/mfx_wavefront.hip b/mafrixraytracing_amd/csrc/mfx_wavefront.hip
--- a/mafrixraytracing_amd/csrc/mfx_wavefront.hip
+++ b/mafrixraytracing_amd/csrc/mfx_wavefront.hip
@@ -628,8 +628,10 @@
         const bool act = j < P.total && x < P.width && y < P.height;
         if (!__any(act)) continue;
         CAM_MARK(t_scan);
+        const bool seen = !(CUTS && MFX_CUT_EMPTY_SKIP) || row->code != MFX_CUT_END;
+        if (act && !seen) c_primary++;
         DV o = dv(0, 0, 0), d = dv(0, 0, 1);
-        if (act) {
+        if (act && seen) {
             const int64_t pixel = (int64_t)x * P.height + y;
             const int64_t gsample = path_gsample<LIST>(P, smp);
             const uint64_t key = path_key(P.seed, (uint64_t)pixel, (uint64_t)gsample);
@@ -645,10 +647,10 @@
         Best B;
 #if MFX_DIAG_STAMPS == 3
         CAM_MARK(t_gen);
-        packet_closest<STATS, true, CUTS>(S, act, o, d, 99999999., B, stk, stm, st, pk_nodes, pk_slots, ph, row, P.cut_cap, &pk_cuts);
+        packet_closest<STATS, true, CUTS>(S, act && seen, o, d, 99999999., B, stk, stm, st, pk_nodes, pk_slots, ph, row, P.cut_cap, &pk_cuts);
         t_last = stamp();
 #else
-        packet_closest<STATS, false, CUTS>(S, act, o, d, 99999999., B, stk, stm, st, pk_nodes, pk_slots, nullptr, row, P.cut_cap,
+        packet_closest<STATS, false, CUTS>(S, act && seen, o, d, 99999999., B, stk, stm, st, pk_nodes, pk_slots, nullptr, row, P.cut_cap,
                                            &pk_cuts);
 #endif
         if (act) {
diff --git a/mafrixraytracing_amd/native.py b/mafrixraytracing_amd/native.py
--- a/mafrixraytracing_amd/native.py
+++ b/mafrixraytracing_amd/native.py
@@ -314,7 +314,8 @@
         check(self.lib.mfx_camera_cut_info(self._h, dptr(out)), "mfx_camera_cut_info")
         return {"builds": int(out[0]), "build_ms": float(out[1]), "len_sum": int(out[2]), "len_max": int(out[3]),
                 "root_tiles": int(out[4]), "empty_tiles": int(out[5]), "tiles": int(out[6]), "cap": int(out[7]),
-                "hist": [int(v) for v in out[8:25]]}
+                "hist": [int(v) for v in out[8:25]], "slots_seen": int(out[25]), "slots_culled": int(out[26]),
+                "leaves_dropped": int(out[27]), "leaves_narrowed": int(out[28]), "culled": bool(out[29])}
 
     def camera_cut_table(self, host: bool = False) -> np.ndarray:
         n = C.c_int64()
```

Result: faster. 12800 Mrays/s (median of 6 runs) (+1.9%).
